# HKU-BAL/MegaPath-Nano

Measured on AMD Instinct MI355X. Metric: Gbp/min ONT reads aligned+species-assigned vs RefSeq, 1/2/4/8 MI355X, higher is better.
Workload: dtype int32

## Files before the change

### megapath_nano_amd/csrc/align.hip

```cpp
#include "map_types.h"
#include "ext_kernels.h"
#include "fin_kernels.h"
#include "tag_kernels.h"
#include "stitch_kernels.h"
#include "plan_kernels.h"
#include "hit_kernels.h"
#include "mapper_internal.h"
#include "../../include/mpn_map.h"
#include "../../include/mpn_ssw.h"

#include <algorithm>
#include <condition_variable>
#include <deque>
#include <math.h>
#include <stdio.h>
#include <string.h>
#include <thread>
#include <pthread.h>
#include <time.h>
#include <atomic>
#include <functional>
#include <mutex>
#include <stdlib.h>
#include <string>
// ... 629 lines not shown
                snprintf(buf, sizeof(buf), ",%d,%d;", q.mapq, q.blen - q.mlen + q.n_ambi);
                out += buf;
            }
        }
        if (r.has_p && o->with_cigar) write_diff_tags(o, r, out);
        snprintf(buf, sizeof(buf), "\trl:i:%d\n", rep_len);
        out += buf;
    }
}

struct Slot {
    hipEvent_t ev_b = nullptr, ev_c = nullptr;
    Arena arena;
    PoolBuf pool_jobs, pool_P, pool_P2, pool_OFF, pool_order, pool_state, pool_CIG, pool_res, pool_redo, pool_compact, pool_used;
    PoolBuf pool_redo_ids, pool_sregs, pool_souts, pool_fin_jobs, pool_fin_out, pool_fin_cig;
    PoolBuf pool_probes, pool_sizes, pool_buckets, pool_pregs, pool_psum, pool_job_anchor, pool_splits, pool_tags;
    PoolBuf pin_segs{nullptr, 0, true}, pin_pregs{nullptr, 0, true}, pin_hits{nullptr, 0, true};
    PoolBuf pin_order{nullptr, 0, true}, pin_res{nullptr, 0, true};
    PoolBuf pin_chain_u{nullptr, 0, true}, pin_chain_b{nullptr, 0, true};
    PoolBuf pin_fin_cig{nullptr, 0, true}, pin_fin_out{nullptr, 0, true}, pin_tags{nullptr, 0, true}, pin_tag_bytes{nullptr, 0, true};
    std::vector<std::vector<SqueezeSeg>> seg_stage;
    size_t device_bytes() const {
        size_t h = 0;
        for (const PoolBuf *pb : {&pool_jobs, &pool_P, &pool_P2, &pool_OFF, &pool_order, &pool_state, &pool_CIG, &pool_res, &pool_redo, &pool_compact, &pool_used,
                                  &pool_redo_ids, &pool_sregs, &pool_souts, &pool_fin_jobs, &pool_fin_out, &pool_fin_cig, &pool_probes, &pool_sizes, &pool_buckets,
                                  &pool_pregs, &pool_psum, &pool_job_anchor, &pool_splits, &pool_tags})
            h += pb->cap;
        for (const auto &c : arena.chunks) h += c.cap;
        return h;
    }
    void release_device() {
        arena.release_all();
        for (PoolBuf *pb : {&pool_jobs, &pool_P, &pool_P2, &pool_OFF, &pool_order, &pool_state, &pool_CIG, &pool_res, &pool_redo, &pool_compact, &pool_used,
                            &pool_redo_ids, &pool_sregs, &pool_souts, &pool_fin_jobs, &pool_fin_out, &pool_fin_cig, &pool_probes, &pool_sizes, &pool_buckets,
                            &pool_pregs, &pool_psum, &pool_job_anchor, &pool_splits, &pool_tags})
            pb->release();
    }
};
static Slot g_slots[16];
static thread_local Slot *tl_slot = &g_slots[0];

static int g_force_kernel = 0;

static void parallel_chunks(int64_t n, int n_threads, const std::function<void(int64_t, int64_t, int)> &fn, int tag = 0) {
    if (n_threads <= 1 || n < 8192) { fn(0, n, 0); return; }
    g_pool.parallel_for(n_threads, n_threads, [&](int t, int) { fn(n * t / n_threads, n * (t + 1) / n_threads, t); }, tag, 1);
}

__global__ void ext_redo_patch_kernel(ExtJob *jobs, const int32_t *ids, const int32_t *layout, const int32_t *qstride,
                                      const int64_t *p_off, const int32_t *inv, int zdrop_inv, int n) {
    const int k = blockIdx.x * blockDim.x + threadIdx.x;
    if (k >= n) return;
    ExtJob &jb = jobs[ids[k]];
    jb.flag &= ~EZ_APPROX_MAX;
    if (inv[k]) { jb.flag |= EZ_INV; jb.zdrop = zdrop_inv; }
    jb.layout = layout[k];
    jb.qstride = qstride[k];
    jb.p_off = p_off[k];
}

__global__ void ref_codes_kernel(RefView rv, const int64_t *g0, const int64_t *off, int n_iv, int8_t *out) {
    for (int k = blockIdx.y; k < n_iv; k += gridDim.y) {
        const int64_t n = off[k + 1] - off[k];
        for (int64_t i = (int64_t)blockIdx.x * blockDim.x + threadIdx.x; i < n; i += (int64_t)gridDim.x * blockDim.x)
            out[off[k] + i] = (int8_t)ref_code(rv, g0[k] + i);
    }
}
struct RefIv { int64_t seq_off; int start, n; };
static int fetch_ref_codes(const RefView &rv, const std::vector<RefIv> &iv, std::vector<std::vector<int8_t>> &out, StreamLease &st) {
    const int n_iv = (int)iv.size();
    out.resize((size_t)n_iv);
    if (n_iv == 0) return 0;
    std::vector<int64_t> tab((size_t)2 * n_iv + 1);
    int64_t *g0 = tab.data(), *off = g0 + n_iv;
    int max_n = 0;
    off[0] = 0;
    for (int k = 0; k < n_iv; ++k) {
        const int n = std::max(0, iv[(size_t)k].n);
        g0[k] = iv[(size_t)k].seq_off + iv[(size_t)k].start;
        off[k + 1] = off[k] + n;
        max_n = std::max(max_n, n);
    }
    const int64_t tot = off[n_iv];
    std::vector<int8_t> codes((size_t)tot);
    if (tot > 0) {
        DevBuf<int64_t> d_tab;
        DevBuf<int8_t> d;
        if (d_tab.alloc(tab.size()) || d.alloc((size_t)tot)) return -1;
        MPN_HIP_CHECK(hipMemcpyAsync(d_tab.p, tab.data(), tab.size() * 8, hipMemcpyHostToDevice, st));
        hipLaunchKernelGGL(ref_codes_kernel, dim3((unsigned)std::min(64, (max_n + 255) / 256), (unsigned)std::min(n_iv, 65535)), dim3(256), 0, st,
                           rv, (const int64_t *)d_tab.p, (const int64_t *)d_tab.p + n_iv, n_iv, d.p);
        MPN_HIP_CHECK(hipGetLastError());
        MPN_HIP_CHECK(hipMemcpyAsync(codes.data(), d.p, (size_t)tot, hipMemcpyDeviceToHost, st));
        MPN_HIP_CHECK(stream_sync(st));
    }
    for (int k = 0; k < n_iv; ++k) out[(size_t)k].assign(codes.begin() + off[k], codes.begin() + off[k + 1]);
    return 0;
}
static inline int8_t host_code(char c) { c |= 0x20; return c == 'a' ? 0 : c == 'c' ? 1 : c == 'g' ? 2 : (c == 't' || c == 'u') ? 3 : 4; }
static inline int8_t host_qbase(const char *seq, int rlen, int rev, int x) {
    if (!rev) return host_code(seq[x]);
    const int8_t c = host_code(seq[rlen - 1 - x]);
    return c < 4 ? (int8_t)(3 - c) : (int8_t)4;
}
struct LocalHit { int score, qe, te; };
static int local_scores(const mpn_map_opt *opt, const std::vector<std::vector<int8_t>> &qs, const std::vector<std::vector<int8_t>> &ts, std::vector<LocalHit> &out) {
    const int n = (int)qs.size();
    out.assign((size_t)n, LocalHit{0, -1, -1});
    if (n == 0) return 0;
    std::vector<int8_t> qb, tb;
    std::vector<int64_t> qo(n), to(n), coff(n);
    std::vector<int32_t> ql(n), tl(n), mask(n, 15), rb(n), re(n), qb1(n), qe1(n), re2(n), clen(n), status(n);
    std::vector<uint16_t> s1(n), s2(n);
    for (int i = 0; i < n; ++i) {
        qo[i] = (int64_t)qb.size(); ql[i] = (int32_t)qs[i].size(); qb.insert(qb.end(), qs[i].begin(), qs[i].end());
        to[i] = (int64_t)tb.size(); tl[i] = (int32_t)ts[i].size(); tb.insert(tb.end(), ts[i].begin(), ts[i].end());
    }
    int8_t mat[25];
    for (int i = 0; i < 4; ++i) { for (int j = 0; j < 4; ++j) mat[i * 5 + j] = (int8_t)(i == j ? opt->a : -opt->b); mat[i * 5 + 4] = (int8_t)-opt->sc_ambi; }
    for (int i = 0; i < 5; ++i) mat[20 + i] = (int8_t)-opt->sc_ambi;
    uint32_t dummy_cig[4];
    const int rc = mpn_ssw_align_batch(n, qb.data(), qo.data(), ql.data(), tb.data(), to.data(), tl.data(), mat, 5, 2, (uint8_t)(opt->q + opt->e), (uint8_t)opt->e,
                                       0, 0, 0, mask.data(), s1.data(), s2.data(), rb.data(), re.data(), qb1.data(), qe1.data(), re2.data(), dummy_cig, 4,
                                       coff.data(), clen.data(), status.data());
    if (rc) return -1;
    for (int i = 0; i < n; ++i) if (status[i] == 0) out[(size_t)i] = LocalHit{(int)s1[i], qe1[i], re[i]};
    return 0;
}

struct DevRound {
    ExtJob *jobs = nullptr;
    ExtRes *res = nullptr;
    uint32_t *compact = nullptr;
    unsigned long long *used = nullptr;
    int64_t cig_cap = 0;
    int n_jobs = 0;
};

struct HostSeqs { const char *seqs; const int64_t *seq_off; const int32_t *seq_len; const int64_t *tseq_off; };

static int run_job_group(const RefView &rv, const mpn_map_opt *opt, int nj_cap, const unsigned long long *d_nj, DevRound &dv, const uint8_t *d_reads,
                         const int64_t *d_read_off, const int32_t *d_read_len, int64_t budget, const HostSeqs *hs, StreamLease &st) {
    if (nj_cap == 0) return 0;
    int nj = nj_cap;
    WallTimer wt;
    Slot &SL = *tl_slot;
    const int strip_scores = ext_strip_scores_ok(opt->a, -opt->b, -opt->sc_ambi, opt->q + opt->e, opt->q2 + opt->e2) ? 1 : 0;
    ExtParams prm;
    prm.sc_mch = (int8_t)opt->a; prm.sc_mis = (int8_t)-opt->b; prm.sc_n = (int8_t)-opt->sc_ambi;
    prm.q = (int8_t)opt->q; prm.e = (int8_t)opt->e; prm.q2 = (int8_t)opt->q2; prm.e2 = (int8_t)opt->e2; prm.zdrop_thres = opt->zdrop;
    prm.zdrop_inv = opt->zdrop_inv; prm.max_gap = opt->max_gap;
    const size_t order_cap = (size_t)nj + (size_t)N_STRIP * 8 + 16;
    if (SL.pool_sizes.ensure((size_t)nj * sizeof(JobSizes) + 16) || SL.pool_buckets.ensure((size_t)2 * N_BUCKETS * 4 + sizeof(LayoutTotals) + 16) ||
        SL.pool_order.ensure(order_cap * 4) || SL.pin_res.ensure(sizeof(LayoutTotals) + 96) ||
        SL.pool_redo_ids.ensure((size_t)nj * 4 + 16) || SL.pool_probes.ensure((size_t)nj * sizeof(InvProbe) + 16))
        return -1;
    struct { ExtJob *p; } d_jobs{dv.jobs};
    JobSizes *d_sizes = SL.pool_sizes.as<JobSizes>();
    int32_t *d_bcnt = SL.pool_buckets.as<int32_t>(), *d_bcur = d_bcnt + N_BUCKETS;
    LayoutTotals *d_tot = reinterpret_cast<LayoutTotals *>(d_bcnt + 2 * N_BUCKETS);
    struct { int32_t *p; } d_order{SL.pool_order.as<int32_t>()};
    {
        ZeroList z{};
        zero_list_push(z, d_bcnt, (size_t)2 * N_BUCKETS * 4 + sizeof(LayoutTotals));
        zero_list_push(z, dv.used + 1, 8);
        zero_list_push(z, dv.used + 5, 8);
        zero_list_push(z, dv.used + 8, 16);
        zero_list_push(z, dv.used + 7, 8);
        MPN_HIP_CHECK(zero_regions(z, st));
    }
    const int lay_grid = std::max(1, std::min((nj + 255) / 256, 256));
    EvTimer evl(st);
    static const bool tiled_on = []() { const char *e = getenv("MPN_TILED"); return !e || atoi(e) != 0; }();
    static const int tile_pick = []() { const char *e = getenv("MPN_TILE_CLASS"); return e ? std::min(std::max(atoi(e), 0), N_TILE_CLASS - 1) : -1; }();
    hipLaunchKernelGGL(job_classify_kernel, dim3(lay_grid), dim3(256), 0, st, d_jobs.p, d_nj, strip_scores, prm, g_force_kernel ? g_force_kernel : (tiled_on ? 0 : 7),
                       tile_pick, d_sizes, d_bcnt, d_tot);
    hipLaunchKernelGGL(job_scan_kernel, dim3(1), dim3(1024), 0, st, d_sizes, d_nj, (const int32_t *)d_bcnt, d_bcur, d_tot, d_order.p);
    hipLaunchKernelGGL(job_layout_kernel, dim3(lay_grid), dim3(256), 0, st, d_jobs.p, d_nj, (const JobSizes *)d_sizes, d_bcur, d_order.p);
    MPN_HIP_CHECK(hipGetLastError());
    LayoutTotals *h_tot = SL.pin_res.as<LayoutTotals>();
    evl.mark(56);
    MPN_HIP_CHECK(hipMemcpyAsync(h_tot, d_tot, sizeof(LayoutTotals), hipMemcpyDeviceToHost, st));
    MPN_HIP_CHECK(stream_sync(st));
    evl.resolve();
    const LayoutTotals T = *h_tot;
    nj = T.n_jobs;
    dv.n_jobs = nj;
    if (nj == 0) return 0;
    if (T.too_large) { set_error("DP window too large for LDS staging (%d x %d)", T.tl_q, T.tl_t); return -4; }
    if (!dv.compact) {
        if (SL.pool_compact.ensure((size_t)T.cig_tot * 4 * 2 + 16)) return -1;
        dv.compact = SL.pool_compact.as<uint32_t>();
        dv.cig_cap = T.cig_tot;
    }
    if (budget > 0 && T.p_tot > budget && nj > 1) return 1;
    const int *cnt = T.cnt, *base = T.base;
    g_stats[4] += nj; g_stats[5] += T.cells; g_stats[31] += T.strip_cells[0] + T.strip_cells[1] + T.strip_cells[2];
    for (int c = 0; c < 3; ++c) g_stats[41 + c] += T.strip_cells[c];
    g_stats[58] += T.xstrip_cells;
    for (int c = 0; c < N_TILE_CLASS; ++c) {
        g_stats[64] += cnt[L_TILE + c];
        g_stats[STAT_TILE_CLASS + c] += cnt[L_TILE + c];
    }
    if (getenv("MPN_DEBUG_JOBS")) {
        static const char *const fam[] = {"wg64", "wg", "strip", "band", "tile"};
        for (int l = 0; l < N_LISTS; ++l)
            if (cnt[l]) fprintf(stderr, "[jobs] %s list %-2d n=%d\n", fam[l < L_WG ? 0 : l < L_STRIP ? 1 : l < L_BAND ? 2 : l < L_TILE ? 3 : 4], l, cnt[l]);
    }
    if (const char *dump = getenv("MPN_DUMP_STRIPS")) {
        const int n_ord = base[L_BAND] - base[L_STRIP];
        std::vector<int32_t> ord(n_ord);
        std::vector<ExtJob> hj(nj);
        MPN_HIP_CHECK(hipMemcpy(ord.data(), d_order.p + base[L_STRIP], (size_t)n_ord * 4, hipMemcpyDeviceToHost));
        MPN_HIP_CHECK(hipMemcpy(hj.data(), d_jobs.p, (size_t)nj * sizeof(ExtJob), hipMemcpyDeviceToHost));
        static std::mutex mu;
        std::lock_guard<std::mutex> lk(mu);
        if (const char *all = getenv("MPN_DUMP_JOBS"))
            if (FILE *f = fopen(all, "ab")) {
                for (int j = 0; j < nj; ++j) {
                    const int32_t rec[6] = {hj[j].cls, hj[j].qlen, hj[j].tlen, hj[j].w, hj[j].flag, hj[j].n_col};
                    fwrite(rec, 4, 6, f);
                }
                fclose(f);
            }
        if (FILE *f = fopen(dump, "ab")) {
            for (int l = L_STRIP; l < L_BAND; ++l)
                for (int k = base[l]; k < base[l + 1]; ++k) {
                    const int jid = ord[k - base[L_STRIP]];
                    const int32_t rec[4] = {strip_glc_of_list(l), jid >= 0 ? hj[jid].qlen : 0, jid >= 0 ? hj[jid].tlen : 0, jid >= 0 ? hj[jid].strip_s : 0};
                    fwrite(rec, 4, 4, f);
                }
            fclose(f);
        }
    }
    if (SL.pool_P.ensure((size_t)T.p_tot + 16) || SL.pool_OFF.ensure((size_t)T.row_tot * 2 * 4 + 16) ||
        SL.pool_state.ensure((size_t)T.state_tot + 16) || SL.pool_CIG.ensure((size_t)T.cig_tot * 4 + 16))
        return -1;
    wt.stop_into(g_stats[27]);
    struct { uint8_t *p; } P{SL.pool_P.as<uint8_t>()};
    struct { int32_t *p; } OFF{SL.pool_OFF.as<int32_t>()};
    struct { int8_t *p; } gstate{SL.pool_state.as<int8_t>()};
    struct { uint32_t *p; } CIG{SL.pool_CIG.as<uint32_t>()};
    struct { ExtRes *p; } d_res{dv.res};
    uint32_t *d_compact = dv.compact;
    unsigned long long *d_used = dv.used;
    int32_t *d_redo_ids = SL.pool_redo_ids.as<int32_t>();
    InvProbe *d_probes = SL.pool_probes.as<InvProbe>();
    auto launch_list = [&](int l, const int32_t *ord, int n, hipStream_t s) -> int {
        if (n == 0) return 0;
        if (l < L_STRIP) {
            const int ntc = (l - L_LDS) / 5;
            const size_t lds = std::max<size_t>((size_t)T.lds_need[(l - L_LDS) % 5], 64);
#define MPN_WG_LAUNCH(NT)                                                                                                             \
            do {                                                                                                                      \
                if (lds > 64 * 1024) MPN_HIP_CHECK(hipFuncSetAttribute((const void *)ext_dp_wg_kernel<NT>, hipFuncAttributeMaxDynamicSharedMemorySize, (int)lds)); \
                hipLaunchKernelGGL(ext_dp_wg_kernel<NT>, dim3(n), dim3(NT), lds, s, d_jobs.p, ord, n, prm, d_reads, d_read_off, d_read_len, \
                                   rv, P.p, OFF.p, gstate.p, d_res.p);                                                                \
            } while (0)
            if (ntc == 0) MPN_WG_LAUNCH(64); else if (ntc == 1) MPN_WG_LAUNCH(256); else if (ntc == 2) MPN_WG_LAUNCH(512); else MPN_WG_LAUNCH(1024);
#undef MPN_WG_LAUNCH
        } else if (l < L_BAND) {
            const int fam = (l - L_STRIP) / 48;
            StripSegs segs;
            segs.n = 0;
            int blocks = 0;
            size_t lds = 0;
            const int c_lo = fam == 0 ? 0 : 3, c_hi = fam == 0 ? 3 : N_STRIP_CLASS;
            for (int glc = 2; glc >= 0; --glc)
                for (int sclass = c_lo + glc; sclass < c_hi; sclass += 3) {
                    const int l0 = L_STRIP + 16 * sclass, nl = base[l0 + 16] - base[l0], per = strip_windows_per_wave(l0);
                    if (nl == 0) continue;
                    const int stride = (std::max(T.strip_lds[sclass], 16) + 3) & ~3;
                    const int nr_stride = fam ? T.strip_nr[sclass] + 16 : 0;
                    lds = std::max(lds, (size_t)stride * per + STRIP_TAB_BYTES + (size_t)per * 8 * nr_stride);
                    segs.s[segs.n++] = StripSeg{blocks, nl, base[l0], stride, nr_stride, glc, sclass >= 6 ? 1 : 0};
                    blocks += nl / per;
                }
            if (blocks == 0) return 0;
#define MPN_STRIP_LAUNCH(EX)                                                                                                          \
            do {                                                                                                                      \
                if (lds > 64 * 1024) MPN_HIP_CHECK(hipFuncSetAttribute((const void *)ext_dp_strip_kernel<EX>, hipFuncAttributeMaxDynamicSharedMemorySize, (int)lds)); \
                hipLaunchKernelGGL(ext_dp_strip_kernel<EX>, dim3(blocks), dim3(64), lds, s, d_jobs.p, (const int32_t *)d_order.p, segs, prm, d_reads, \
                                   d_read_off, d_read_len, rv, P.p, d_res.p);                                                         \
            } while (0)
            if (fam == 0) MPN_STRIP_LAUNCH(false); else MPN_STRIP_LAUNCH(true);
#undef MPN_STRIP_LAUNCH
        } else if (l >= L_TILE) {
            const int c = l - L_TILE;
            const size_t lds = (size_t)std::max(T.tile_lds[c], 64);
#define MPN_TILE_LAUNCH(S, NW)                                                                                                        \
            do {                                                                                                                      \
                if (lds > 64 * 1024) MPN_HIP_CHECK(hipFuncSetAttribute((const void *)ext_dp_tile_kernel<S, NW>, hipFuncAttributeMaxDynamicSharedMemorySize, (int)lds)); \
                hipLaunchKernelGGL((ext_dp_tile_kernel<S, NW>), dim3(n), dim3(64 * NW), lds, s, d_jobs.p, ord, n, prm, d_reads, d_read_off, \
                                   d_read_len, rv, P.p, gstate.p, d_res.p, d_used + 7);                                              \
            } while (0)
            static_assert(N_TILE_CLASS == 4, "tile classes");
            if (c == 0) MPN_TILE_LAUNCH(16, 1); else if (c == 1) MPN_TILE_LAUNCH(4, 8); else if (c == 2) MPN_TILE_LAUNCH(8, 4); else MPN_TILE_LAUNCH(4, 16);
#undef MPN_TILE_LAUNCH
        } else {
            const int bvar = (l - L_BAND) / 4;
            const size_t lds = std::max<size_t>((size_t)T.band_lds[(l - L_BAND) % 4], 64);
#define MPN_BAND_LAUNCH(NW, TT)                                                                                                       \
            do {                                                                                                                      \
                if (lds > 64 * 1024) MPN_HIP_CHECK(hipFuncSetAttribute((const void *)ext_dp_band_kernel<NW, TT>, hipFuncAttributeMaxDynamicSharedMemorySize, (int)lds)); \
                hipLaunchKernelGGL((ext_dp_band_kernel<NW, TT>), dim3(n), dim3(NW * 64), lds, s, d_jobs.p, ord, n, prm, d_reads, d_read_off, \
                                   d_read_len, rv, P.p, d_res.p);                                                                    \
            } while (0)
            if (bvar == 0) MPN_BAND_LAUNCH(1, 2); else if (bvar == 1) MPN_BAND_LAUNCH(2, 2); else if (bvar == 2) MPN_BAND_LAUNCH(4, 2); else MPN_BAND_LAUNCH(8, 2);
#undef MPN_BAND_LAUNCH
        }
        MPN_HIP_CHECK(hipGetLastError());
        return 0;
    };
    EvTimer ev(st);
    if (!SL.ev_b) {
        MPN_HIP_CHECK(hipEventCreateWithFlags(&SL.ev_b, hipEventDisableTiming));
        MPN_HIP_CHECK(hipEventCreateWithFlags(&SL.ev_c, hipEventDisableTiming));
    }
    auto on_side = [](int l) { return (l >= L_WG && l < L_STRIP) || l >= L_BAND + 8; };
    bool have_tiles = false;
    for (int l = L_TILE; l < N_LISTS; ++l) have_tiles = have_tiles || cnt[l] > 0;
    bool have_side = false;
    for (int l = 0; l < L_TILE; ++l) have_side = have_side || (on_side(l) && cnt[l] > 0);
    hipStream_t extra[2] = {nullptr, nullptr};
    const int n_extra = st.try_extra((int)have_side + (int)have_tiles, extra);
    if (have_side || have_tiles) ++g_stats[n_extra ? STAT_SIDE_LEASED : STAT_SIDE_OWN];
    const hipStream_t main_st = st;
    const hipStream_t side_st = have_side && n_extra > 0 ? extra[0] : main_st;
    const hipStream_t tile_st = have_tiles && n_extra > (int)have_side ? extra[(int)have_side] : main_st;
    for (int l = L_TILE; l < N_LISTS && have_tiles; ++l)
        if (launch_list(l, d_order.p + base[l], cnt[l], tile_st)) return -1;
    for (int l = L_TILE - 1; l >= 0; --l)
        if (on_side(l) && launch_list(l, d_order.p + base[l], cnt[l], side_st)) return -1;
    const int side_lo[2] = {base[L_WG], base[L_BAND + 8]}, side_hi[2] = {base[L_STRIP], base[L_TILE]};
    const int tile_lo[2] = {base[L_TILE], 0}, tile_hi[2] = {base[N_LISTS], 0};
    const int main_lo[2] = {0, base[L_STRIP]}, main_hi[2] = {base[L_WG], base[L_BAND + 8]};
    static const int walk_mode = []() {
        const char *e = getenv("MPN_EXT_WALK");
        return !e || !strcmp(e, "auto") ? 0 : !strcmp(e, "lane") ? 1 : !strcmp(e, "wave") ? 2 : 0;
    }();
    auto launch_bt = [&](const int32_t *ord, int n, hipStream_t s, bool wave) {
        if (n <= 0) return;
        if (wave) hipLaunchKernelGGL(ext_bt_wave_kernel, dim3(n), dim3(64), 0, s, d_jobs.p, ord, n, P.p, OFF.p, CIG.p, d_compact, d_used, d_res.p, d_used + 8);
        else hipLaunchKernelGGL(ext_bt_kernel, dim3((n + 63) / 64), dim3(64), 0, s, d_jobs.p, ord, n, P.p, OFF.p, CIG.p, d_compact, d_used, d_res.p);
    };
    auto bt_ztest = [&](const int *lo, const int *hi, hipStream_t s, bool timed, bool wave) -> int {
        for (int k = 0; k < 2; ++k) launch_bt(d_order.p + lo[k], hi[k] - lo[k], s, wave);
        MPN_HIP_CHECK(hipGetLastError());
        if (timed) ev.mark(25);
        for (int k = 0; k < 2; ++k) {
            const int n = hi[k] - lo[k];
            if (n <= 0) continue;
            if (wave) hipLaunchKernelGGL(ext_ztest_wave_kernel, dim3(n), dim3(64), 0, s, d_jobs.p, d_order.p + lo[k], n, prm, d_reads, d_read_off, d_read_len, rv, CIG.p, d_res.p,
                                         d_redo_ids, d_used + 1, d_probes, d_used + 5, d_used + 9);
            else hipLaunchKernelGGL(ext_ztest_kernel, dim3((n + 63) / 64), dim3(64), 0, s, d_jobs.p, d_order.p + lo[k], n, prm, d_reads, d_read_off, d_read_len, rv, CIG.p, d_res.p,
                                    d_redo_ids, d_used + 1, d_probes, d_used + 5);
        }
        MPN_HIP_CHECK(hipGetLastError());
        if (timed) ev.mark(26);
        return 0;
    };
    if (have_side || have_tiles) ev.mark(15);
    if (have_tiles) {
        if (bt_ztest(tile_lo, tile_hi, tile_st, false, walk_mode != 1)) return -1;
        if (tile_st != main_st) MPN_HIP_CHECK(hipEventRecord(SL.ev_c, tile_st));
    }
    if (bt_ztest(side_lo, side_hi, side_st, false, walk_mode != 1)) return -1;
    if (side_st != main_st) MPN_HIP_CHECK(hipEventRecord(SL.ev_b, side_st));
    if (have_side || have_tiles) ev.mark(STAT_EV_WALK_LONG);
    for (int l = N_LISTS - 1; l >= 0; --l) {
        if (on_side(l)) continue;
        if (l == L_BAND - 1) ev.mark(15);
        if (l >= L_STRIP && l < L_BAND) {
            if (l == L_STRIP + 48) { if (launch_list(l, nullptr, 1, main_st)) return -1; ev.mark(57); }
            else if (l == L_STRIP) { if (launch_list(l, nullptr, 1, main_st)) return -1; ev.mark(9, 38); }
        } else if (launch_list(l, d_order.p + base[l], cnt[l], main_st)) return -1;
    }
    ev.mark(15);
    if (bt_ztest(main_lo, main_hi, main_st, true, walk_mode == 2)) return -1;
    if (side_st != main_st) MPN_HIP_CHECK(hipStreamWaitEvent(main_st, SL.ev_b, 0));
    if (tile_st != main_st) MPN_HIP_CHECK(hipStreamWaitEvent(main_st, SL.ev_c, 0));
    unsigned long long *h_used = reinterpret_cast<unsigned long long *>(reinterpret_cast<char *>(SL.pin_res.p) + ((sizeof(LayoutTotals) + 15) & ~(size_t)15));
    MPN_HIP_CHECK(hipMemcpyAsync(h_used, d_used, 80, hipMemcpyDeviceToHost, st));
    wt.stop_into(g_stats[28]);
    MPN_HIP_CHECK(stream_sync(st));
    wt.stop_into(g_stats[29]);
    g_stats[STAT_WALK_WAVE] += (int64_t)h_used[8];
    g_stats[STAT_WALK_WAVE_FAILED] += (int64_t)h_used[9];
    if (h_used[7]) {
        g_stats[STAT_TILE_GIVEUPS] += (int64_t)h_used[7];
        set_error("%llu tiled DP windows gave up waiting for their hand-off", (unsigned long long)h_used[7]);
        return -1;
    }
    std::vector<int32_t> redo((size_t)h_used[1]);
    const int n_probe = (int)h_used[5];
    if (!redo.empty() || n_probe) {
        std::vector<ExtJob> jobs((size_t)nj);
        std::vector<InvProbe> probes((size_t)n_probe);
        if (SL.pin_order.ensure(redo.size() * 4 + 16)) return -1;
        if (!redo.empty()) MPN_HIP_CHECK(hipMemcpyAsync(SL.pin_order.p, d_redo_ids, redo.size() * 4, hipMemcpyDeviceToHost, st));
        MPN_HIP_CHECK(hipMemcpyAsync(jobs.data(), d_jobs.p, (size_t)nj * sizeof(ExtJob), hipMemcpyDeviceToHost, st));
        if (n_probe) MPN_HIP_CHECK(hipMemcpyAsync(probes.data(), d_probes, (size_t)n_probe * sizeof(InvProbe), hipMemcpyDeviceToHost, st));
        MPN_HIP_CHECK(stream_sync(st));
        if (!redo.empty()) memcpy(redo.data(), SL.pin_order.p, redo.size() * 4);
        std::vector<uint8_t> is_inv((size_t)nj, 0);
        if (n_probe) {
            std::sort(probes.begin(), probes.end(), [](const InvProbe &x, const InvProbe &y) { return x.jid < y.jid; });
            std::vector<LocalHit> hits((size_t)n_probe, LocalHit{0, -1, -1});
            if (hs) {
                std::vector<std::vector<int8_t>> qv((size_t)n_probe), tv;
                std::vector<RefIv> iv((size_t)n_probe);
                for (int k = 0; k < n_probe; ++k) {
                    const InvProbe &pb = probes[(size_t)k];
                    const ExtJob &jb = jobs[(size_t)pb.jid];
                    const int q_len = pb.q1 - pb.q0, t_len = pb.t1 - pb.t0, rlen = hs->seq_len[jb.read];
                    const char *rd = hs->seqs + hs->seq_off[jb.read];
                    qv[(size_t)k].resize((size_t)q_len);
                    for (int x = 0; x < q_len; ++x) { const int8_t c = host_qbase(rd, rlen, jb.rev, jb.qs + pb.q1 - x - 1); qv[(size_t)k][(size_t)x] = c >= 4 ? (int8_t)4 : (int8_t)(3 - c); }
                    iv[(size_t)k] = RefIv{hs->tseq_off[jb.rid], jb.ts + pb.t0, t_len};
                }
                if (fetch_ref_codes(rv, iv, tv, st)) return -1;
                if (local_scores(opt, qv, tv, hits)) return -1;
            }
            for (int k = 0; k < n_probe; ++k) {
                const InvProbe &pb = probes[(size_t)k];
                const bool inv = hits[(size_t)k].score >= opt->min_chain_score * opt->a && hits[(size_t)k].score >= opt->min_dp_max;
                if (inv) is_inv[(size_t)pb.jid] = 1;
                if (inv || pb.over) redo.push_back(pb.jid);
            }
        }
        g_stats[8] += (int64_t)redo.size();
        const int nr = (int)redo.size();
        auto list_of = [&](int j) { return jobs[(size_t)j].cls & 0xff; };
        auto redo_list_of = [&](int j) { return jobs[(size_t)j].cls >> 8 & 0xff; };
        auto band_of = [&](int j) { return (jobs[(size_t)j].cls >> 16 & 0xff) - 1; };
        std::sort(redo.begin(), redo.end(), [&](int x, int y) { return redo_list_of(x) != redo_list_of(y) ? redo_list_of(x) < redo_list_of(y) : x < y; });
        std::vector<int32_t> pack((size_t)nr * 6 + 2);
        const size_t off_p = ((size_t)nr * 4 + 1) & ~(size_t)1;
        int64_t *pack_off = reinterpret_cast<int64_t *>(pack.data() + off_p);
        int64_t p2_tot = 0;
        for (int k = 0; k < nr; ++k) {
            const int j = redo[k];
            const ExtJob &jb = jobs[(size_t)j];
            const int bv = band_of(j);
            pack[k] = j; pack[nr + k] = bv >= 0 ? 2 : 0; pack[2 * nr + k] = 128 << std::max(bv, 0); pack[3 * nr + k] = is_inv[(size_t)j];
            if ((list_of(j) >= L_STRIP && list_of(j) < L_BAND) || list_of(j) >= L_TILE) {
                const int64_t n_r = (int64_t)jb.qlen + jb.tlen - 1;
                pack_off[k] = -1 - p2_tot;
                p2_tot += ((bv >= 0 ? n_r * (128 << bv) : n_r * jb.n_col) + 15) & ~(int64_t)15;
            } else pack_off[k] = jb.p_off;
        }
        if (nr > 0) {
            if (SL.pool_P2.ensure((size_t)p2_tot + 16)) return -1;
            const int64_t p2_base = (int64_t)(SL.pool_P2.as<uint8_t>() - P.p);
            for (int k = 0; k < nr; ++k) if (pack_off[k] < 0) pack_off[k] = p2_base + (-1 - pack_off[k]);
            if (SL.pool_redo.ensure(pack.size() * 4)) return -1;
            struct { int32_t *p; } d_redo{SL.pool_redo.as<int32_t>()};
            MPN_HIP_CHECK(hipMemcpyAsync(d_redo.p, pack.data(), pack.size() * 4, hipMemcpyHostToDevice, st));
            hipLaunchKernelGGL(ext_redo_patch_kernel, dim3((nr + 255) / 256), dim3(256), 0, st, d_jobs.p, d_redo.p, d_redo.p + nr, d_redo.p + 2 * nr,
                               reinterpret_cast<const int64_t *>(d_redo.p + off_p), d_redo.p + 3 * nr, opt->zdrop_inv, nr);
            MPN_HIP_CHECK(hipGetLastError());
            ev.skip();
            for (int lo = 0; lo < nr;) {
                int hi = lo;
                while (hi < nr && redo_list_of(redo[hi]) == redo_list_of(redo[lo])) ++hi;
                if (launch_list(redo_list_of(redo[lo]), d_redo.p + lo, hi - lo, st)) return -1;
                lo = hi;
            }
            ev.mark(15);
            launch_bt(d_redo.p, nr, st, walk_mode == 2);
            if (walk_mode == 2) g_stats[STAT_WALK_WAVE] += nr;
            MPN_HIP_CHECK(hipGetLastError());
            ev.mark(25);
            MPN_HIP_CHECK(stream_sync(st));
        }
    }
    ev.resolve();
    wt.stop_into(g_stats[30]);
    return 0;
}

static int run_jobs(const RefView &rv, const mpn_map_opt *opt, int nj_cap, const uint8_t *d_reads, const int64_t *d_read_off,
                    const int32_t *d_read_len, DevRound &out, const HostSeqs *hs, StreamLease &st, bool block_zeroed = false) {
    static const int64_t budget = []() { const char *e = getenv("MPN_DP_BUDGET"); return e ? std::max<int64_t>(1 << 20, atoll(e)) : (int64_t)40 << 30; }();
    Slot &SL = *tl_slot;
    if (SL.pool_res.ensure((size_t)nj_cap * sizeof(ExtRes) + 16) || SL.pool_used.ensure(128)) return -1;
    out.jobs = SL.pool_jobs.as<ExtJob>(); out.res = SL.pool_res.as<ExtRes>(); out.compact = nullptr;
    out.used = SL.pool_used.as<unsigned long long>();
    if (!block_zeroed) {
        MPN_HIP_CHECK(hipMemsetAsync(out.used, 0, 24, st));
        MPN_HIP_CHECK(hipMemsetAsync(out.used + 5, 0, 24, st));
    }
    const int rc = run_job_group(rv, opt, nj_cap, out.used + 3, out, d_reads, d_read_off, d_read_len, budget, hs, st);
    if (rc != 1) return rc;
    const int nj = out.n_jobs;
    std::vector<JobSizes> sz((size_t)nj);
    MPN_HIP_CHECK(hipMemcpyAsync(sz.data(), SL.pool_sizes.p, (size_t)nj * sizeof(JobSizes), hipMemcpyDeviceToHost, st));
    MPN_HIP_CHECK(stream_sync(st));
    std::vector<int> cuts{0};
    for (int j = 1; j < nj; ++j) if (sz[(size_t)j].p - sz[(size_t)cuts.back()].p > budget) cuts.push_back(j);
    cuts.push_back(nj);
    for (size_t g = 0; g + 1 < cuts.size(); ++g) {
        DevRound dv = out;
        dv.jobs += cuts[g]; dv.res += cuts[g];
        const unsigned long long cnt = (unsigned long long)(cuts[g + 1] - cuts[g]);
        MPN_HIP_CHECK(hipMemcpyAsync(out.used + 4, &cnt, 8, hipMemcpyHostToDevice, st));
        const int r2 = run_job_group(rv, opt, (int)cnt, out.used + 4, dv, d_reads, d_read_off, d_read_len, 0, hs, st);
        if (r2) return r2 < 0 ? r2 : -1;
    }
    out.n_jobs = nj;
    return 0;
}

}

using namespace mpn;

static int plan_enqueue(const mpn_map_opt *opt, int32_t k, const PlanReg *d_pr, int n_sr, u128 *d_a, const int32_t *d_tlens,
                        unsigned long long *d_used, ExtJob *d_jobs, int32_t *d_janchor, StitchReg *d_sr, PlanSum *d_ps, int grid_cap,
                        hipStream_t st) {
    PlanOpt po;
    po.bw = opt->bw; po.bw15 = (int)(opt->bw * 1.5 + 1.); po.min_chain_score = opt->min_chain_score; po.max_gap = opt->max_gap;
    po.min_cnt = opt->min_cnt; po.a = opt->a; po.q = opt->q; po.e = opt->e; po.zdrop = opt->zdrop; po.zdrop_inv = opt->zdrop_inv;
    po.end_bonus = opt->end_bonus; po.min_ksw_len = opt->min_ksw_len; po.k = k; po.pad = 0; po.max_sw_mat = opt->max_sw_mat;
    MPN_HIP_CHECK(hipMemsetAsync(d_used, 0, 64, st));
    int grid = std::min(n_sr, 256 * 4);
    if (grid_cap > 0) grid = std::min(grid, grid_cap);
    hipLaunchKernelGGL(plan_kernel, dim3((unsigned)grid), dim3(64), 0, st, po, d_pr, n_sr, d_a, d_tlens, d_used + 3, d_jobs, d_janchor, d_sr, d_ps);
    MPN_HIP_CHECK(hipGetLastError());
    return 0;
}

static bool g_need_cigar = true;

struct RoundDev {
    const StitchReg *sregs; const PlanReg *pregs; const PlanSum *psum; const int32_t *job_anchor; const u128 *anchors;
};

static int stitch_enqueue(const RoundDev &rd, int n_sr, const ExtJob *d_jobs, const ExtRes *d_res, const uint32_t *d_compact, uint32_t *d_cig,
                          unsigned long long *d_out_used, StitchOut *d_so, FinJob *d_fj, int min_cnt, SplitRec *d_splits,
                          unsigned long long *d_n_splits, int grid_cap, hipStream_t st) {
// ... 1840 lines not shown
```

### megapath_nano_amd/csrc/ext_kernels.h

```cpp
#pragma once
#include "mpn_common.h"
#include "map_types.h"

namespace mpn {

enum { EZ_APPROX_MAX = 0x02, EZ_RIGHT = 0x08, EZ_EXTZ_ONLY = 0x40, EZ_REV_CIGAR = 0x80 };

struct ExtJob {
    int32_t read;
    int32_t rid;
    int32_t rev;
    int32_t qs, qlen;
    int32_t ts, tlen;
    int32_t reversed;
    int32_t w, zdrop, end_bonus, flag;
    int64_t p_off;
    int64_t row_off;
    int64_t cig_off;
    int32_t n_col;
    int32_t state_mode;
    int64_t state_off;
    int32_t layout;
    int32_t qstride;
    int32_t strip_s;
// ... 752 lines not shown
        uint32_t Vp = ((uint32_t)v_s & nh) | (((uint32_t)bj * both + CV) & ~nh), X1 = (uint32_t)x1_s & nh, X2 = (uint32_t)x2_s & nh;
        if (j >= 0 && j < qmax && gl < nlmax) {
            uint32_t dwa[(S + 3) / 4], dwb[(S + 3) / 4], ecell[4] = {0, 0, 0, 0};
            uint32_t nv0 = 0;
#pragma unroll
            for (int k = 0; k < S; ++k) {
                const uint32_t sc = __builtin_amdgcn_perm(qta, KONST, T1[k]) | __builtin_amdgcn_perm(qtb, KONST, T2[k]);
                const uint32_t Up = U[k];
                const uint32_t A1 = X1 + Vp, A2 = X2 + Vp, B1 = Y1[k] + Up, B2 = Y2[k] + Up;
                const uint32_t M1 = __builtin_bit_cast(uint32_t, __builtin_elementwise_max(__builtin_bit_cast(s16x2, A1), __builtin_bit_cast(s16x2, B1)));
                const uint32_t M2 = __builtin_bit_cast(uint32_t, __builtin_elementwise_max(__builtin_bit_cast(s16x2, A2), __builtin_bit_cast(s16x2, B2))) - DD;
                const uint32_t M = __builtin_bit_cast(uint32_t, __builtin_elementwise_max(__builtin_bit_cast(s16x2, M1), __builtin_bit_cast(s16x2, M2)));
                const uint32_t z = __builtin_bit_cast(uint32_t, __builtin_elementwise_max(__builtin_bit_cast(s16x2, M), __builtin_bit_cast(s16x2, sc)));
                const uint32_t zc = __builtin_bit_cast(uint32_t, __builtin_elementwise_min(__builtin_bit_cast(s16x2, z), __builtin_bit_cast(s16x2, MCH7)));
                const uint32_t Zc = zc & RANK_CLR;
                const uint32_t ZZ = Zc + KZZ;
                uint32_t nu = Up, nv;
                asm("v_sub_u32 %1, %2, %0\n\tv_sub_u32 %0, %2, %3" : "+v"(nu), "=&v"(nv) : "v"(ZZ), "v"(Vp));
                const u16x2 An1 = __builtin_elementwise_sub_sat(__builtin_bit_cast(u16x2, A1), __builtin_bit_cast(u16x2, Zc + KEA1));
                const u16x2 An2 = __builtin_elementwise_sub_sat(__builtin_bit_cast(u16x2, A2), __builtin_bit_cast(u16x2, Zc + KEA2));
                const u16x2 Bn1 = __builtin_elementwise_sub_sat(__builtin_bit_cast(u16x2, B1), __builtin_bit_cast(u16x2, Zc + KEB1));
                const u16x2 Bn2 = __builtin_elementwise_sub_sat(__builtin_bit_cast(u16x2, B2), __builtin_bit_cast(u16x2, Zc + KEB2));
                uint32_t HA1, HB1, HA2, HB2, F;
                asm("v_pk_min_u16 %0, %1, %2" : "=v"(HA1) : "v"(__builtin_bit_cast(uint32_t, An1)), "v"(EIGHT));
                asm("v_pk_min_u16 %0, %1, %2" : "=v"(HB1) : "v"(__builtin_bit_cast(uint32_t, Bn1)), "v"(EIGHT));
                asm("v_pk_min_u16 %0, %1, %2" : "=v"(HA2) : "v"(__builtin_bit_cast(uint32_t, An2)), "v"(EIGHT));
                asm("v_pk_min_u16 %0, %1, %2" : "=v"(HB2) : "v"(__builtin_bit_cast(uint32_t, Bn2)), "v"(EIGHT));
                asm("v_lshl_or_b32 %0, %1, 1, %2" : "=v"(F) : "v"(HB1), "v"(HA1));
                asm("v_lshl_or_b32 %0, %1, 2, %2" : "=v"(F) : "v"(HA2), "v"(F));
                asm("v_lshl_or_b32 %0, %1, 3, %2" : "=v"(F) : "v"(HB2), "v"(F));
                asm("v_and_or_b32 %0, %1, %2, %3" : "=v"(ecell[k & 3]) : "v"(z), "v"(SEVEN), "v"(F));
                U[k] = nu; Y1[k] = __builtin_bit_cast(uint32_t, Bn1); Y2[k] = __builtin_bit_cast(uint32_t, Bn2);
                Vp = nv; X1 = __builtin_bit_cast(uint32_t, An1); X2 = __builtin_bit_cast(uint32_t, An2);
                if ((k & 3) == 3 || k == S - 1) {
                    const uint32_t p01 = (k & 3) >= 1 ? __builtin_amdgcn_perm(ecell[1], ecell[0], 0x06020400u) : __builtin_amdgcn_perm(0u, ecell[0], 0x0c020c00u);
                    const uint32_t p23 = (k & 3) == 3 ? __builtin_amdgcn_perm(ecell[3], ecell[2], 0x06020400u)
                                       : (k & 3) == 2 ? __builtin_amdgcn_perm(0u, ecell[2], 0x0c020c00u) : 0u;
                    dwa[k >> 2] = __builtin_amdgcn_perm(p23, p01, 0x05040100u);
                    dwb[k >> 2] = __builtin_amdgcn_perm(p23, p01, 0x07060302u);
                }
                if (k == 0) nv0 = nv;
            }
            out_v = (int)Vp; out_x1 = (int)X1; out_x2 = (int)X2;
            if (j <= qa1) row0a += (int)(nv0 & 0xffffu) - cv1;
            if (j <= qb1) row0b += (int)(nv0 >> 16) - cv1;
            auto packed_sum = [&]() -> uint32_t {
                u16x2 acc = __builtin_bit_cast(u16x2, U[0]);
#pragma unroll
                for (int k = 1; k < S; ++k) acc += __builtin_bit_cast(u16x2, U[k]);
                return __builtin_bit_cast(uint32_t, acc);
            };
            if (j == qa1) {
                if (!head && t0 + S <= tlen[0]) tota += (int)(short)(uint16_t)((packed_sum() & 0xffffu) - (uint32_t)(S * cu1));
                else {
#pragma unroll
                    for (int k = 0; k < S; ++k) tota += (t0 + k > 0 && t0 + k < tlen[0]) ? (int)(U[k] & 0xffffu) - cu1 : 0;
                }
            }
            if (j == qb1) {
                if (!head && t0 + S <= tlen[1]) totb += (int)(short)(uint16_t)((packed_sum() >> 16) - (uint32_t)(S * cu1));
                else {
#pragma unroll
                    for (int k = 0; k < S; ++k) totb += (t0 + k > 0 && t0 + k < tlen[1]) ? (int)(U[k] >> 16) - cu1 : 0;
                }
            }
            auto store = [&](uint8_t *dst, const uint32_t *dw) {
                if constexpr (S == 4) *reinterpret_cast<uint32_t *>(dst) = dw[0];
                else if constexpr (S == 8) *reinterpret_cast<uint2 *>(dst) = make_uint2(dw[0], dw[1]);
                else if constexpr (S == 16) *reinterpret_cast<uint4 *>(dst) = make_uint4(dw[0], dw[1], dw[2], dw[3]);
                else {
#pragma unroll
                    for (int c = 0; c < S / 4; ++c) __builtin_memcpy(dst + 4 * c, &dw[c], 4);
                    if constexpr ((S & 2) != 0) { const uint16_t h = (uint16_t)dw[S / 4]; __builtin_memcpy(dst + (S & ~3), &h, 2); }
                    if constexpr ((S & 1) != 0) dst[S - 1] = (uint8_t)(dw[S / 4] >> ((S & 2) ? 16 : 0));
                }
            };
            if (j <= qa1 && gl < nl0) store(prow0 + (int64_t)step * W[0], dwa);
            if (j <= qb1 && gl < nl1) store(prow1 + (int64_t)step * W[1], dwb);
        }
    }
#undef MPN_BND
    int32_t ta = tota + (head ? row0a - 8 * qe : 0), tb = totb + (head ? row0b - 8 * qe : 0);
#pragma unroll
    for (int dlt = GL / 2; dlt; dlt >>= 1) { ta += __shfl_xor(ta, dlt); tb += __shfl_xor(tb, dlt); }
    ta >>= 3; tb >>= 3;
    if (head) {
#pragma unroll
        for (int w = 0; w < 2; ++w) {
            if (jid[w] < 0) continue;
            ExtRes out;
            out.max = 0; out.zdropped = 0; out.max_q = out.max_t = out.mqe_t = -1; out.mqe = NEG_INF; out.score = ok[w] ? (w ? tb : ta) : NEG_INF;
            out.reach_end = 0; out.n_cigar = 0; out.r_done = ok[w] ? qlen[w] + tlen[w] - 2 : -1; out.zcode = 0; out.cig_pos = 0;
            out.do_bt = ok[w] ? 1 : 0; out.bt_i = ok[w] ? tlen[w] - 1 : -1; out.bt_j = ok[w] ? qlen[w] - 1 : -1;
            res[jid[w]] = out;
        }
    }
}

template <int GL, bool RIGHT>
__device__ __forceinline__ void ext_strip_exact_dispatch(const ExtJob *__restrict__ jobs, const int32_t *__restrict__ order, const int first,
                                                         const int n_list, const ExtParams &prm, const uint8_t *__restrict__ reads,
                                                         const int64_t *__restrict__ read_off, const int32_t *__restrict__ read_len,
                                                         const RefView &rv, uint8_t *__restrict__ P, ExtRes *__restrict__ res, uint8_t *smem,
                                                         const int lds_stride, const int nr_stride) {
    const int j0 = first < n_list ? order[first] : -1;
    if (j0 < 0) return;
    const int S = jobs[j0].strip_s;
#define MPN_CASE(SS) case SS: ext_strip_exact<SS, GL, RIGHT>(jobs, order, first, n_list, prm, reads, read_off, read_len, rv, P, res, smem, lds_stride, nr_stride); break
    switch (S) {
        MPN_CASE(1); MPN_CASE(2); MPN_CASE(3); MPN_CASE(4); MPN_CASE(5); MPN_CASE(6); MPN_CASE(7); MPN_CASE(8);
        MPN_CASE(9); MPN_CASE(10); MPN_CASE(11); MPN_CASE(12); MPN_CASE(13); MPN_CASE(14); MPN_CASE(15);
        default: ext_strip_exact<16, GL, RIGHT>(jobs, order, first, n_list, prm, reads, read_off, read_len, rv, P, res, smem, lds_stride, nr_stride); break;
    }
#undef MPN_CASE
}

struct StripSeg { int32_t first_block, n_list, ord_off, lds_stride, nr_stride, glc, right; };
struct StripSegs { StripSeg s[6]; int32_t n; };

template <bool EXACT>
__global__ __launch_bounds__(64) __attribute__((amdgpu_waves_per_eu(3, 3))) void ext_dp_strip_kernel(const ExtJob *__restrict__ jobs, const int32_t *__restrict__ order, StripSegs segs,
                                                          ExtParams prm, const uint8_t *__restrict__ reads,
                                                          const int64_t *__restrict__ read_off, const int32_t *__restrict__ read_len,
                                                          RefView rv, uint8_t *__restrict__ P, ExtRes *__restrict__ res) {
    extern __shared__ __attribute__((aligned(16))) uint8_t smem[];
    int k = 0;
    while (k + 1 < segs.n && (int)blockIdx.x >= segs.s[k + 1].first_block) ++k;
    const StripSeg sg = segs.s[k];
    const int32_t *ord = order + sg.ord_off;
    if constexpr (!EXACT) {
        {
            const int first2 = ((int)blockIdx.x - sg.first_block) * (8 >> sg.glc);
            int S = 16;
            for (int k = 0; k < (8 >> sg.glc); ++k) { const int slot = first2 + k; if (slot < sg.n_list && ord[slot] >= 0) { S = jobs[ord[slot]].strip_s; break; } }
#define MPN_PAIR(SS, GLN) ext_strip_pair<SS, GLN>(jobs, ord, first2, sg.n_list, prm, reads, read_off, read_len, rv, P, res, smem, sg.lds_stride)
#define MPN_PAIR_S(GLN) switch (S) { case 1: MPN_PAIR(1, GLN); break; case 2: MPN_PAIR(2, GLN); break; case 3: MPN_PAIR(3, GLN); break; case 4: MPN_PAIR(4, GLN); break; \
            case 5: MPN_PAIR(5, GLN); break; case 6: MPN_PAIR(6, GLN); break; case 7: MPN_PAIR(7, GLN); break; case 8: MPN_PAIR(8, GLN); break; \
            case 9: MPN_PAIR(9, GLN); break; case 10: MPN_PAIR(10, GLN); break; case 11: MPN_PAIR(11, GLN); break; case 12: MPN_PAIR(12, GLN); break; \
            case 13: MPN_PAIR(13, GLN); break; case 14: MPN_PAIR(14, GLN); break; case 15: MPN_PAIR(15, GLN); break; default: MPN_PAIR(16, GLN); break; }
            if (sg.glc == 0) MPN_PAIR_S(16) else if (sg.glc == 1) MPN_PAIR_S(32) else MPN_PAIR_S(64)
#undef MPN_PAIR_S
#undef MPN_PAIR
        }
    } else {
        const int first = ((int)blockIdx.x - sg.first_block) * (4 >> sg.glc);
#define MPN_GL(GLN, RT) ext_strip_exact_dispatch<GLN, RT>(jobs, ord, first, sg.n_list, prm, reads, read_off, read_len, rv, P, res, smem, sg.lds_stride, sg.nr_stride)
        if (sg.right) { if (sg.glc == 0) MPN_GL(16, true); else if (sg.glc == 1) MPN_GL(32, true); else MPN_GL(64, true); }
        else { if (sg.glc == 0) MPN_GL(16, false); else if (sg.glc == 1) MPN_GL(32, false); else MPN_GL(64, false); }
#undef MPN_GL
    }
}

struct TileGeom { int T0, rows, n_lanes, W, jlo, jhi; int64_t base; };
__host__ __device__ inline TileGeom tile_geom(int tile, int qlen, int tlen, int w, int S) {
    const int R = 64 * S;
    TileGeom g{};
    g.T0 = tile * R;
    g.rows = tlen - g.T0 < R ? tlen - g.T0 : R;
    g.n_lanes = (g.rows + S - 1) / S;
    g.W = g.n_lanes * S;
    g.jlo = g.T0 - w > 0 ? g.T0 - w : 0;
    g.jhi = g.T0 + g.rows - 1 + w < qlen - 1 ? g.T0 + g.rows - 1 + w : qlen - 1;
    const int64_t m = tile;
    const int64_t k0 = (int64_t)w / R + 1;
    const int64_t n0 = m > k0 ? m - k0 : 0;
    const int64_t s_lo = (int64_t)R * (n0 * (k0 + m - 1) / 2) - n0 * (int64_t)w;
    const int64_t num = (int64_t)qlen - R - w;
    int64_t k1 = num <= 0 ? 0 : (num + R - 1) / R;
    if (k1 > m) k1 = m;
    const int64_t s_hi = (int64_t)R * (k1 * (k1 - 1) / 2) + k1 * (int64_t)(R - 1 + w) + (m - k1) * (int64_t)(qlen - 1);
    g.base = (s_hi - s_lo + 64 * m) * R;
    return g;
}
__host__ __device__ inline int64_t tile_matrix_bytes(int qlen, int tlen, int w, int S) {
    const int R = 64 * S, nt_all = (tlen + R - 1) / R, nt_band = (int)(((int64_t)qlen - 1 + w) / R) + 1, nt = nt_all < nt_band ? nt_all : nt_band;
    const TileGeom g = tile_geom(nt - 1, qlen, tlen, w, S);
    return g.base + (int64_t)((g.jhi >= g.jlo ? g.jhi - g.jlo + 1 : 0) + g.n_lanes - 1) * g.W;
}
__host__ __device__ inline bool ext_tile_ok(int qlen, int tlen, int w) {
    const int d = qlen > tlen ? qlen - tlen : tlen - qlen;
    return qlen > 0 && tlen > 0 && w >= 1 && d <= w && tlen <= 32768 && qlen <= 60000;
}

__host__ __device__ inline bool ext_tile_exact_ok(int mch, int mis, int amb, int q, int e, int q2, int e2, int qlen, int tlen, int w) {
    if (!(qlen > 0 && tlen > 0 && w >= 1 && tlen <= 8191 && qlen <= 16384 && qlen + tlen - 1 <= 14000)) return false;
    const int mn = qlen < tlen ? qlen : tlen, mx = qlen > tlen ? qlen : tlen;
    int worst = mis < amb ? -mis : -amb;
    if (worst < 0) worst = 0;
    const int g1 = worst * mn + q + e * (mx - mn + 1), g1b = q + e * (mx + 1), g2 = worst * mn + q2 + e2 * (mx - mn + 1), g2b = q2 + e2 * (mx + 1);
    const int lo1 = g1 > g1b ? g1 : g1b, lo2 = g2 > g2b ? g2 : g2b;
    return mch * mn < 32000 && (lo1 < lo2 ? lo1 : lo2) < 32000;
}
constexpr int TILE_RING_COLS = 2048, TILE_CTRL_BYTES = 4 * (2 * 16 + 4);
__host__ __device__ inline int ext_tile_ring_off(int qlen) { return ((qlen + 3) & ~3) + 64 + TILE_CTRL_BYTES; }
__host__ __device__ inline int ext_tile_lds_bytes(int qlen, int tlen, bool exact, int NW) {
    return ext_tile_ring_off(qlen) + (NW > 1 ? 12 * TILE_RING_COLS : 0) + (exact ? 8 * ((qlen + tlen + 2) & ~3) : 0);
}
__host__ __device__ inline bool ext_tile_pipe_ok(int w, int S, int NW) {
    return 2 * w + 128 < NW * (TILE_RING_COLS / NW + 64 * S);
}
constexpr int TILE_SPIN_MAX = 1 << 21;

template <int S, int NW, bool EXACT, bool RIGHT>
__device__ __forceinline__ void ext_tile_body(const ExtJob &jb, const int jid, const ExtParams &prm, const uint8_t *__restrict__ reads,
                                              const int64_t *__restrict__ read_off, const int32_t *__restrict__ read_len, const RefView &rv,
                                              uint8_t *__restrict__ P, int8_t *__restrict__ gstate, ExtRes *__restrict__ res, uint8_t *smem,
                                              unsigned long long *__restrict__ n_failed) {
    static_assert(S % 4 == 0 && S <= 16 && NW >= 1 && NW <= 16, "rows per lane: 4, 8, 12 or 16");
    constexpr int R = 64 * S, NT = 64 * NW;
    const int tid = threadIdx.x, lane = tid & 63, wave = tid >> 6;
    const int qlen = jb.qlen, tlen = jb.tlen;
    int q = prm.q, e = prm.e, q2 = prm.q2, e2 = prm.e2;
    if (q2 + e2 < q + e) { int t_ = q; q = q2; q2 = t_; t_ = e; e = e2; e2 = t_; }
    const int qe = q + e, qe2 = q2 + e2;
    int w = jb.w;
    if (w < 0) w = tlen > qlen ? tlen : qlen;
    ExtRes out;
    out.max = 0; out.zdropped = 0; out.max_q = out.max_t = out.mqe_t = -1; out.mqe = NEG_INF; out.score = NEG_INF;
    out.reach_end = 0; out.n_cigar = 0; out.r_done = -1; out.bt_i = out.bt_j = -1; out.do_bt = 0; out.zcode = 0; out.cig_pos = 0;
    if (!(EXACT ? ext_tile_exact_ok(prm.sc_mch, prm.sc_mis, prm.sc_n, prm.q, prm.e, prm.q2, prm.e2, qlen, tlen, w) : ext_tile_ok(qlen, tlen, w)) || -prm.sc_mis > 2 * (q + e) ||
        (NW > 1 && !ext_tile_pipe_ok(w, S, NW))) { if (tid == 0) res[jid] = out; return; }
    constexpr int RS = RIGHT ? 0 : 4, RA = RIGHT ? 1 : 3, RB = 2, RA2 = RIGHT ? 3 : 1, RB2 = RIGHT ? 4 : 0;
    const uint32_t sb_mch = (uint32_t)(8 * prm.sc_mch + RS + 128) & 0xff, sb_mis = (uint32_t)(8 * prm.sc_mis + RS + 128) & 0xff,
                   sb_n = (uint32_t)(8 * prm.sc_n + RS + 128) & 0xff;
    const int q_pad = (qlen + 3) & ~3;
    uint32_t *tab = reinterpret_cast<uint32_t *>(smem + q_pad);
    if (tid < 5) tab[tid] = lane == 4 ? sb_n * 0x01010101u : (sb_mis * 0x01010101u) ^ ((sb_mch ^ sb_mis) << (8 * lane));
    {
        const int64_t roff = read_off[jb.read];
        const int32_t rlen = read_len[jb.read];
        for (int i = tid; i < qlen; i += NT) smem[i] = (uint8_t)(4 * ext_qbase(reads, roff, rlen, jb.rev, jb.qs + (jb.reversed ? qlen - 1 - i : i)));
    }
    int long_thres = e != e2 ? (q2 - q) / (e - e2) - 1 : 0;
    if (q2 + e2 + long_thres * e2 > q + e + long_thres * e) ++long_thres;
    const int long_diff = long_thres * (e - e2) - (q2 - q) - e2;
#define MPN_BND(R) (8 * ((R) == 0 ? -qe : (R) < long_thres ? -e : (R) == long_thres ? long_diff : -e2))
    typedef short s16x2 __attribute__((ext_vector_type(2)));
    typedef unsigned short u16x2 __attribute__((ext_vector_type(2)));
    auto pk = [](int lo, int hi) { return (uint32_t)(hi * 65536 + lo); };
    constexpr int BETA = 0x2000 + 128;
    const int cv_lo = -8 * qe + RA + BETA, cv_hi = -8 * qe2 + RA2 + BETA, cu_lo = -8 * qe + RB + BETA, cu_hi = -8 * qe2 + RB2 + BETA;
    const uint32_t CV = pk(cv_lo, cv_hi), CU = pk(cu_lo, cu_hi);
    const uint32_t FRESH_U = pk(-8 * qe, -8 * qe) + CU, EDGE_V = pk(-8 * qe, -8 * qe) + CV;
    const uint32_t KONST = sb_n | 0x2000u;
    const uint32_t KZZ = pk(-16 * qe + RA + RB + BETA, -16 * qe2 + RA2 + RB2 + BETA);
    constexpr int RU = RIGHT ? 8 : 0;
    const uint32_t KEA = pk(8 * e - 8 * qe + RA - RU, 8 * e2 - 8 * qe2 + RA2 - RU), KEB = pk(8 * e - 8 * qe + RB - RU, 8 * e2 - 8 * qe2 + RB2 - RU);
    const uint32_t EIGHT = 0x00080008u, RANK_CLR = 0xfff8fff8u;
    const uint32_t MCH7 = (uint32_t)(8 * prm.sc_mch + 7 + BETA) * 0x00010001u;
    const int64_t g0 = rv.seq_off[jb.rid] + jb.ts;
    uint32_t *bnd_base = reinterpret_cast<uint32_t *>(gstate + jb.state_off);
    const int n_tiles = (tlen + R - 1) / R;
    uint32_t *ctrl = reinterpret_cast<uint32_t *>(smem + ext_tile_ring_off(qlen) - TILE_CTRL_BYTES);
    uint32_t *ring = ctrl + TILE_CTRL_BYTES / 4;
    constexpr int C = TILE_RING_COLS / NW;
    const int n_r = qlen + tlen - 1;
    uint32_t *BEST = reinterpret_cast<uint32_t *>(smem + ext_tile_ring_off(qlen) + (NW > 1 ? 12 * TILE_RING_COLS : 0)), *SE = BEST + ((n_r + 3) & ~3);
    int32_t *HL = reinterpret_cast<int32_t *>(NW > 1 ? bnd_base : bnd_base + 6 * (size_t)qlen);
    if (tid < 2 * NW + 1) ctrl[tid] = 0;
    if constexpr (EXACT) {
        for (int r = tid; r < n_r; r += NT) {
            int st = 0, en = tlen - 1;
            if (st < r - qlen + 1) st = r - qlen + 1;
            if (en > r) en = r;
            if (st < (r - w + 1) >> 1) st = (r - w + 1) >> 1;
            if (en > (r + w) >> 1) en = (r + w) >> 1;
            if (st > en) { st = 1; en = 0; }
            BEST[r] = 0;
            SE[r] = (uint32_t)st | (uint32_t)en << 16;
        }
        for (int t = tid; t < tlen; t += NT) HL[t] = NEG_INF;
        __builtin_amdgcn_fence(__ATOMIC_RELEASE, "agent");
    }
    __syncthreads();
    const bool head = lane == 0;
    int32_t score8 = 0;
    uint32_t *const prod_in = &ctrl[(wave + NW - 1) % NW], *const cons_in = &ctrl[NW + (wave + NW - 1) % NW];
    uint32_t *const prod_out = &ctrl[wave], *const cons_out = &ctrl[NW + wave];
    uint32_t *const ring_in = ring + 3 * C * ((wave + NW - 1) % NW), *const ring_out = ring + 3 * C * wave;
    uint32_t n_in = 0, n_out = 0, seen_prod = 0, seen_cons = 0;
    bool failed = false;
    auto wait_gt = [&](uint32_t *ctr, uint32_t lim, uint32_t &seen) -> bool {
        if ((int)(seen - lim) > 0) return true;
        for (int k = 0; k < TILE_SPIN_MAX; ++k) {
            seen = __hip_atomic_load(ctr, __ATOMIC_RELAXED, __HIP_MEMORY_SCOPE_WORKGROUP);
            if ((int)(seen - lim) > 0) return true;
            if (__hip_atomic_load(&ctrl[2 * NW], __ATOMIC_RELAXED, __HIP_MEMORY_SCOPE_WORKGROUP)) return false;
            __builtin_amdgcn_s_sleep(1);
        }
        __hip_atomic_store(&ctrl[2 * NW], 1u, __ATOMIC_RELAXED, __HIP_MEMORY_SCOPE_WORKGROUP);
        return false;
    };
    for (int tile = NW > 1 ? wave : 0; tile < n_tiles; tile += NW) {
        const TileGeom G = tile_geom(tile, qlen, tlen, w, S);
        const int T0 = G.T0, n_lanes = G.n_lanes, W = G.W, jlo = G.jlo, jhi = G.jhi;
        if (jhi < jlo) break;
        const int prev_jhi = tile > 0 ? min(qlen - 1, T0 - 1 + w) : -1;
        const int jlo_next = T0 + R - w > 0 ? T0 + R - w : 0;
        uint32_t *bnd_in = bnd_base + (size_t)(tile & 1) * 3 * (size_t)qlen, *bnd_out = bnd_base + (size_t)((tile + 1) & 1) * 3 * (size_t)qlen;
        const bool write_bnd = tile + 1 < n_tiles;
        const int t0 = T0 + lane * S;
        uint32_t UL[S], YL[S], TSEL[S];
        int32_t H8[S];
#pragma unroll
        for (int k = 0; k < S; ++k) {
            const int t = t0 + k;
            const int sq = t < tlen ? ref_code(rv, g0 + (jb.reversed ? tlen - 1 - t : t)) : 4;
            TSEL[k] = 0x0c0c0100u | (sq < 4 ? 4u + (uint32_t)sq : 0u);
            UL[k] = jlo == 0 ? pk(MPN_BND(t), MPN_BND(t)) + CU : FRESH_U;
            YL[k] = 0;
            H8[k] = 8 * (t < long_thres ? -(q + e * (t + 1)) : -(q2 + e2 * (t + 1)));
        }
        uint8_t *prow = P + jb.p_off + G.base + (int64_t)lane * S;
        const int n_steps = (jhi - jlo + 1) + n_lanes - 1;
        int out_v = 0, out_x = 0, out_h = 0;
        uint32_t qt = 0;
        auto qcode = [&](int col) -> uint32_t { return col < qlen ? (uint32_t)smem[col] : 16u; };
        uint32_t qt_next = *reinterpret_cast<const uint32_t *>(reinterpret_cast<const uint8_t *>(tab) + qcode(jlo));
        uint32_t qc_next = qcode(jlo + 1);
        uint32_t bv_n = 0, bx_n = 0, bh_n = 0, bv_n2 = 0, bx_n2 = 0, bh_n2 = 0;
        auto load_bnd = [&](int col, uint32_t &a, uint32_t &b, uint32_t &c) {
            if (tile > 0 && head && col <= prev_jhi && col < qlen) {
                if constexpr (NW == 1) { a = bnd_in[3 * (size_t)col]; b = bnd_in[3 * (size_t)col + 1]; c = bnd_in[3 * (size_t)col + 2]; }
                else {
                    const uint32_t n = n_in + (uint32_t)(col - jlo), slot = n % C;
                    if (!failed && !wait_gt(prod_in, n, seen_prod)) failed = true;
                    __atomic_signal_fence(__ATOMIC_SEQ_CST);
                    a = ring_in[slot]; b = ring_in[C + slot]; c = ring_in[2 * C + slot];
                    __atomic_signal_fence(__ATOMIC_SEQ_CST);
                    __hip_atomic_store(cons_in, n + 1, __ATOMIC_RELAXED, __HIP_MEMORY_SCOPE_WORKGROUP);
                }
            }
        };
        load_bnd(jlo, bv_n, bx_n, bh_n);
        load_bnd(jlo + 1, bv_n2, bx_n2, bh_n2);
        for (int step = 0; step < n_steps; ++step) {
            const uint32_t q_in = qt_next;
            qt_next = *reinterpret_cast<const uint32_t *>(reinterpret_cast<const uint8_t *>(tab) + qc_next);
            qc_next = qcode(jlo + step + 2);
            const uint32_t bv = bv_n, bx = bx_n, bh = bh_n;
            bv_n = bv_n2; bx_n = bx_n2; bh_n = bh_n2;
            load_bnd(jlo + step + 2, bv_n2, bx_n2, bh_n2);
            const uint32_t qt_s = (uint32_t)wave_shr1_zero((int)qt);
            const int v_s = wave_shr1_zero(out_v), x_s = wave_shr1_zero(out_x), h_s = wave_shr1_zero(out_h);
            const int j = jlo + step - lane;
            qt = head ? q_in : qt_s;
            uint32_t Vp, Xp;
            int32_t Hup;
            if (head) {
                if (tile == 0) { const int bj = MPN_BND(j); Vp = pk(bj, bj) + CV; Xp = 0; Hup = 0; }
                else { Vp = bv; Xp = bx; Hup = (int32_t)bh; }
            } else { Vp = (uint32_t)v_s; Xp = (uint32_t)x_s; Hup = h_s; }
            if (j >= jlo && j <= jhi && lane < n_lanes) {
                uint32_t dw[S / 4], ecell[4] = {0, 0, 0, 0};
                const int d_in = j - t0 + w;
                const int d_out = j - t0 - w;
#pragma unroll
                for (int k = 0; k < S; ++k) {
                    const bool enter = d_in == k, edge = d_out == k;
                    const uint32_t Up = enter ? FRESH_U : UL[k];
                    const uint32_t Yl = enter ? 0u : YL[k];
                    Vp = edge ? EDGE_V : Vp;
                    Xp = edge ? 0u : Xp;
                    const uint32_t sc16 = __builtin_amdgcn_perm(qt, KONST, TSEL[k]);
                    const uint32_t A = Xp + Vp, B = Yl + Up;
                    const uint32_t M = __builtin_bit_cast(uint32_t, __builtin_elementwise_max(__builtin_bit_cast(s16x2, A), __builtin_bit_cast(s16x2, B)));
                    uint32_t m2, z16;
                    asm("v_pk_max_i16 %0, %1, %1 op_sel:[0,1] op_sel_hi:[1,0]" : "=v"(m2) : "v"(M));
                    asm("v_max_i16 %0, %1, %2" : "=v"(z16) : "v"(m2), "v"(sc16));
                    uint32_t zc;
                    asm("v_pk_min_i16 %0, %1, %2 op_sel_hi:[0,1]" : "=v"(zc) : "v"(z16), "v"(MCH7));
                    const uint32_t Zc = zc & RANK_CLR;
                    const uint32_t ZZ = Zc + KZZ;
                    const uint32_t nu = ZZ - Vp, nv = ZZ - Up;
                    u16x2 An = __builtin_elementwise_sub_sat(__builtin_bit_cast(u16x2, A), __builtin_bit_cast(u16x2, Zc + KEA));
                    u16x2 Bn = __builtin_elementwise_sub_sat(__builtin_bit_cast(u16x2, B), __builtin_bit_cast(u16x2, Zc + KEB));
                    uint32_t HA, HB;
                    asm("v_pk_min_u16 %0, %1, %2" : "=v"(HA) : "v"(__builtin_bit_cast(uint32_t, An)), "v"(EIGHT));
                    asm("v_pk_min_u16 %0, %1, %2" : "=v"(HB) : "v"(__builtin_bit_cast(uint32_t, Bn)), "v"(EIGHT));
                    if constexpr (RIGHT) {
                        An = __builtin_elementwise_sub_sat(An, __builtin_bit_cast(u16x2, EIGHT));
                        Bn = __builtin_elementwise_sub_sat(Bn, __builtin_bit_cast(u16x2, EIGHT));
                    }
                    uint32_t Fw;
                    asm("v_lshl_or_b32 %0, %1, 1, %2" : "=v"(Fw) : "v"(HB), "v"(HA));
                    asm("v_and_or_b32 %0, %1, 7, %2" : "=v"(ecell[k & 3]) : "v"(z16), "v"(Fw));
                    const int32_t h_left = H8[k] + (int32_t)(nv & 0xffffu) - cv_lo, h_up = Hup + (int32_t)(nu & 0xffffu) - cu_lo;
                    const int32_t h = enter ? h_up : h_left;
                    H8[k] = h;
                    Hup = h;
                    if constexpr (EXACT) {
                        const int t = t0 + k, r = t + j;
                        const uint32_t se = SE[r < n_r ? r : n_r - 1];
                        const int st_ = (int)(se & 0xffffu), en_ = (int)(se >> 16);
                        const bool inb = t >= st_ && t <= en_;
                        const int en1 = st_ + ((en_ - st_) & ~3);
                        const int cls = t == en_ ? 0 : t < en1 ? 1 + ((t - st_) & 3) : 5;
                        const uint32_t word = (uint32_t)((h >> 3) + 32768) << 16 | (0xffffu - ((uint32_t)cls << 13 | (uint32_t)t));
                        atomicMax(&BEST[r < n_r ? r : n_r - 1], inb ? word : 0u);
                        if (inb && j == qlen - 1) HL[t] = h >> 3;
                    }
                    UL[k] = nu; YL[k] = __builtin_bit_cast(uint32_t, Bn);
                    Vp = nv; Xp = __builtin_bit_cast(uint32_t, An);
                    if ((k & 3) == 3) {
                        uint32_t e01, e23;
                        asm("v_lshl_or_b32 %0, %1, 8, %2" : "=v"(e01) : "v"(ecell[1]), "v"(ecell[0]));
                        asm("v_lshl_or_b32 %0, %1, 8, %2" : "=v"(e23) : "v"(ecell[3]), "v"(ecell[2]));
                        const uint32_t lo = __builtin_amdgcn_perm(e23, e01, 0x05040100u), hi = __builtin_amdgcn_perm(e23, e01, 0x07060302u);
                        asm("v_lshl_or_b32 %0, %1, 2, %2" : "=v"(dw[k >> 2]) : "v"(hi), "v"(lo));
                    }
                }
                out_v = (int)Vp; out_x = (int)Xp; out_h = Hup;
                if constexpr (S == 16) *reinterpret_cast<uint4 *>(prow + (int64_t)step * W) = make_uint4(dw[0], dw[1], dw[2], dw[3]);
                else if constexpr (S == 8) *reinterpret_cast<uint2 *>(prow + (int64_t)step * W) = make_uint2(dw[0], dw[1]);
                else if constexpr (S == 4) *reinterpret_cast<uint32_t *>(prow + (int64_t)step * W) = dw[0];
                if constexpr (NW == 1) {
                    if (write_bnd && lane == 63) { bnd_out[3 * (size_t)j] = (uint32_t)out_v; bnd_out[3 * (size_t)j + 1] = (uint32_t)out_x; bnd_out[3 * (size_t)j + 2] = (uint32_t)out_h; }
                } else if (write_bnd && lane == 63 && j >= jlo_next) {
                    const uint32_t n = n_out + (uint32_t)(j - jlo_next), slot = n % C;
                    if (!failed && !wait_gt(cons_out, n - C, seen_cons)) failed = true;
                    __atomic_signal_fence(__ATOMIC_SEQ_CST);
                    ring_out[slot] = (uint32_t)out_v; ring_out[C + slot] = (uint32_t)out_x; ring_out[2 * C + slot] = (uint32_t)out_h;
                    __atomic_signal_fence(__ATOMIC_SEQ_CST);
                    __hip_atomic_store(prod_out, n + 1, __ATOMIC_RELAXED, __HIP_MEMORY_SCOPE_WORKGROUP);
                }
            }
        }
        if (tile + 1 == n_tiles) {
            const int lt = tlen - 1 - T0, ll = lt / S, kk = lt % S;
            int32_t hv = 0;
#pragma unroll
            for (int k = 0; k < S; ++k) hv = k == kk ? H8[k] : hv;
            score8 = __shfl(hv, ll);
        }
        if constexpr (NW == 1) {
            __builtin_amdgcn_fence(__ATOMIC_RELEASE, "agent");
            __syncthreads();
            __builtin_amdgcn_fence(__ATOMIC_ACQUIRE, "agent");
        } else {
            if (tile > 0 && prev_jhi >= jlo) n_in += (uint32_t)(prev_jhi - jlo + 1);
            if (write_bnd && jhi >= jlo_next) n_out += (uint32_t)(jhi - jlo_next + 1);
        }
    }
#undef MPN_BND
    if constexpr (NW > 1) {
        __builtin_amdgcn_fence(__ATOMIC_RELEASE, "agent");
        __syncthreads();
        __builtin_amdgcn_fence(__ATOMIC_ACQUIRE, "agent");
        if (wave != (EXACT ? 0 : (n_tiles - 1) % NW)) return;
        if (__hip_atomic_load(&ctrl[2 * NW], __ATOMIC_RELAXED, __HIP_MEMORY_SCOPE_WORKGROUP)) {
            if (lane == 0) { res[jid] = out; atomicAdd(n_failed, 1ull); }
            return;
        }
    }
    if constexpr (!EXACT) {
        if (lane == 0) {
            out.score = score8 >> 3;
            out.r_done = qlen + tlen - 2;
            out.do_bt = 1; out.bt_i = tlen - 1; out.bt_j = qlen - 1;
            res[jid] = out;
        }
    } else {
        if constexpr (NW == 1) __syncthreads();
        const int tlm1 = tlen - 1;
        struct Best { int m, t, r; };
        auto scan_first_max = [&](Best x) {
#pragma unroll
            for (int d = 1; d < 64; d <<= 1) {
                const Best o{__shfl_up(x.m, d), __shfl_up(x.t, d), __shfl_up(x.r, d)};
                if (lane >= d && !(x.m > o.m)) x = o;
            }
            return x;
        };
        auto diag = [&](int r, int &H, int &mt) {
            const uint32_t pv = BEST[r];
            H = pv ? (int)(pv >> 16) - 32768 : NEG_INF;
            mt = (int)((0xffffu - (pv & 0xffffu)) & 8191u);
        };
        int r_lim = n_r;
        for (int r = lane; r < n_r; r += 64) { const uint32_t se = SE[r]; if ((int)(se & 0xffffu) > (int)(se >> 16)) { r_lim = r; break; } }
        r_lim = wave_reduce_min(r_lim);
        const int n_eff = r_lim < n_r ? r_lim : n_r;
        const int C = (n_eff + 63) / 64, rlo = min(n_eff, lane * C), rhi = min(n_eff, rlo + C);
        auto chunk_best = [&](int lim) {
            Best b{NEG_INF, -1, -1};
            for (int r = rlo; r < rhi && r <= lim; ++r) { int H, mt; diag(r, H, mt); if (H > b.m) b = Best{H, mt, r}; }
            return b;
        };
        Best incl = scan_first_max(chunk_best(n_eff));
        Best in{__shfl_up(incl.m, 1), __shfl_up(incl.t, 1), __shfl_up(incl.r, 1)};
        ExtApply ez; ez.max = 0; ez.max_t = ez.max_q = -1; ez.zdropped = 0;
        if (lane > 0 && in.m > 0) { ez.max = in.m; ez.max_t = in.t; ez.max_q = in.r - in.t; }
        int r_break = n_eff;
        for (int r = rlo; r < rhi; ++r) {
            int H, mt; diag(r, H, mt);
            if (ext_apply_zdrop(ez, H, r, mt, jb.zdrop, e2)) { r_break = r; break; }
        }
        r_break = wave_reduce_min(r_break);
        const bool zd = r_break < n_eff;
        const bool dropped = zd || n_eff < n_r;
        const int r_last = zd ? r_break : n_eff - 1;
        Best fin = scan_first_max(chunk_best(r_last));
        fin = Best{__shfl(fin.m, 63), __shfl(fin.t, 63), __shfl(fin.r, 63)};
        __builtin_amdgcn_fence(__ATOMIC_ACQUIRE, "agent");
        const int t_lim = min(tlm1, r_last - (qlen - 1));
        const int Ct = (tlen + 63) / 64, tlo = min(tlen, lane * Ct), thi = min(tlen, tlo + Ct);
        Best me{NEG_INF, -1, -1};
        for (int t = tlo; t < thi && t <= t_lim; ++t) { const int h = HL[t]; if (h > me.m) me = Best{h, t, t}; }
        me = scan_first_max(me);
        me = Best{__shfl(me.m, 63), __shfl(me.t, 63), 0};
        if (lane == 0) {
            if (fin.m > 0) { out.max = fin.m; out.max_t = fin.t; out.max_q = fin.r - fin.t; }
            out.zdropped = dropped ? 1 : 0;
            if (me.m > NEG_INF) { out.mqe = me.m; out.mqe_t = me.t; }
            if (!dropped) out.score = HL[tlm1];
            out.r_done = dropped ? (zd ? r_break : n_eff) : n_r - 1;
            if (!dropped && !(jb.flag & EZ_EXTZ_ONLY)) { out.do_bt = 1; out.bt_i = tlen - 1; out.bt_j = qlen - 1; }
            else if (!dropped && (jb.flag & EZ_EXTZ_ONLY) && out.mqe + jb.end_bonus > out.max) { out.reach_end = 1; out.do_bt = 1; out.bt_i = out.mqe_t; out.bt_j = qlen - 1; }
            else if (out.max_t >= 0 && out.max_q >= 0) { out.do_bt = 1; out.bt_i = out.max_t; out.bt_j = out.max_q; }
            res[jid] = out;
        }
    }
}

template <int S, int NW>
__global__ __launch_bounds__(64 * NW) void ext_dp_tile_kernel(const ExtJob *__restrict__ jobs, const int32_t *__restrict__ order, int n_jobs,
                                                              ExtParams prm, const uint8_t *__restrict__ reads,
                                                              const int64_t *__restrict__ read_off, const int32_t *__restrict__ read_len,
                                                              RefView rv, uint8_t *__restrict__ P, int8_t *__restrict__ gstate, ExtRes *__restrict__ res,
                                                              unsigned long long *__restrict__ n_failed) {
    extern __shared__ __attribute__((aligned(16))) uint8_t smem[];
    const int jid = order[blockIdx.x];
    const ExtJob jb = jobs[jid];
#define MPN_TB(EX, RT) ext_tile_body<S, NW, EX, RT>(jb, jid, prm, reads, read_off, read_len, rv, P, gstate, res, smem, n_failed)
    if (jb.flag & EZ_APPROX_MAX) MPN_TB(false, false);
    else if (jb.flag & EZ_RIGHT) MPN_TB(true, true);
    else MPN_TB(true, false);
#undef MPN_TB
}



__device__ __forceinline__ void ext_bt_band(int rr, int qlen, int tlen, int bw, int &st, int &en) {
    st = 0; en = tlen - 1;
    if (st < rr - qlen + 1) st = rr - qlen + 1;
    if (en > rr) en = rr;
    if (st < (rr - bw + 1) >> 1) st = (rr - bw + 1) >> 1;
    if (en > (rr + bw) >> 1) en = (rr + bw) >> 1;
}
__device__ __forceinline__ int ext_bt_force(int i, int st, int en) {
    int force_state = -1;
    if (i < st) force_state = 2;
    if (i > en) force_state = 1;
    return force_state;
}
__device__ __forceinline__ int ext_bt_decode(int b, bool rank_is_op) { return rank_is_op ? b : (b & ~7) | (4 - (b & 7)); }
__device__ __forceinline__ int ext_bt_next_state(int state, int tmp, int force_state) {
    if (state == 0) state = tmp & 7;
    else if (!(tmp >> (state + 2) & 1)) state = 0;
    if (state == 0) state = tmp & 7;
    if (force_state >= 0) state = force_state;
    return state;
}

__global__ __launch_bounds__(64) void ext_bt_kernel(const ExtJob *__restrict__ jobs, const int32_t *__restrict__ order, int n_jobs,
                                                    const uint8_t *__restrict__ P, const int32_t *__restrict__ OFF,
                                                    uint32_t *__restrict__ CIG, uint32_t *__restrict__ COMPACT,
                                                    unsigned long long *__restrict__ compact_used, ExtRes *__restrict__ res) {
    const int k = blockIdx.x * blockDim.x + threadIdx.x;
    const int jid = k < n_jobs ? order[k] : -1;
    const bool live = jid >= 0;
    ExtJob jb = jobs[live ? jid : 0];
    ExtRes r = res[live ? jid : 0];
    const bool walk = live && r.do_bt;
    if (live && !r.do_bt) res[jid].cig_pos = 0;
    if (!walk) { jb.qlen = jb.tlen = 1; r.bt_i = r.bt_j = -1; }
    const int n_col = jb.n_col, n_r = jb.qlen + jb.tlen - 1;
    const uint8_t *p = P + jb.p_off;
    const int32_t *off = OFF + 2 * jb.row_off, *off_end = off + n_r;
    const bool rowmajor = jb.layout == 1;
    const bool rank_is_op = (jb.flag & EZ_RIGHT) != 0;
    const bool byslot = jb.layout == 2;
    const bool tiled = jb.layout == 3;
    TileGeom tg{};
    int tg_tile = -1;
    const int bw = jb.w < 0 ? (jb.tlen > jb.qlen ? jb.tlen : jb.qlen) : jb.w;
    const bool rev_cigar = (jb.flag & EZ_REV_CIGAR) != 0;
    uint32_t *cend = CIG + jb.cig_off;
    const int cap = jb.qlen + jb.tlen + 2;
    uint32_t *cbeg = cend - cap;
    int n = 0, i = r.bt_i, j = r.bt_j, state = 0;
    uint32_t cur_op = 0xf, cur_len = 0;
#define MPN_FLUSH() do { if (cur_len) { if (rev_cigar) cbeg[n] = cur_len << 4 | cur_op; else cend[-1 - n] = cur_len << 4 | cur_op; ++n; } } while (0)
#define MPN_PUSHOP(OP, LEN) do { if ((uint32_t)(OP) == cur_op) cur_len += (LEN); else { MPN_FLUSH(); cur_op = (OP); cur_len = (LEN); } } while (0)
    constexpr int BT_AHEAD = 8;
    while (i >= 0 && j >= 0) {
        const int rr = i + j;
        int force_state = -1, tmp;
        if (rowmajor) {
            if (state == 0) {
                uint8_t ahead[BT_AHEAD];
#pragma unroll
                for (int k = 0; k < BT_AHEAD; ++k) {
                    const int ii = i - k, jj = j - k;
                    ahead[k] = (ii >= 0 && jj >= 0) ? p[(int64_t)(jj + ii / jb.strip_s) * jb.qstride + ii] : (uint8_t)0xff;
                }
                int k = 0;
                tmp = 0;
#pragma unroll
                for (int q = 0; q < BT_AHEAD; ++q) {
                    if (k != q) continue;
                    if (i - q < 0 || j - q < 0) continue;
                    const int b = ext_bt_decode(ahead[q], rank_is_op);
                    if ((b & 7) == 0) ++k; else tmp = b;
                }
                if (k > 0) { MPN_PUSHOP(0, (uint32_t)k); i -= k; j -= k; }
                if (k == BT_AHEAD || i < 0 || j < 0) continue;
            } else {
                tmp = ext_bt_decode(p[(int64_t)(j + i / jb.strip_s) * jb.qstride + i], rank_is_op);
            }
        }
        else if (tiled) {
            int st, en;
            ext_bt_band(rr, jb.qlen, jb.tlen, bw, st, en);
            force_state = ext_bt_force(i, st, en);
            tmp = 0;
            if (force_state < 0) {
                const int tile = i / (64 * jb.strip_s);
                if (tile != tg_tile) { tg = tile_geom(tile, jb.qlen, jb.tlen, bw, jb.strip_s); tg_tile = tile; }
                const int lt = i - tg.T0;
                tmp = ext_bt_decode(p[tg.base + (int64_t)((j - tg.jlo) + lt / jb.strip_s) * tg.W + lt], rank_is_op);
            }
        }
        else if (byslot) {
            int st, en;
            ext_bt_band(rr, jb.qlen, jb.tlen, bw, st, en);
            force_state = ext_bt_force(i, st, en);
            tmp = force_state < 0 ? p[(int64_t)rr * jb.qstride + (i & (jb.qstride - 1))] : 0;
        } else {
            force_state = ext_bt_force(i, off[rr], off_end[rr]);
            tmp = force_state < 0 ? p[(int64_t)rr * n_col + i - off[rr]] : 0;
        }
        state = ext_bt_next_state(state, tmp, force_state);
        if (state == 0) { MPN_PUSHOP(0, 1); --i; --j; }
        else if (state == 1 || state == 3) { MPN_PUSHOP(2, 1); --i; }
        else { MPN_PUSHOP(1, 1); --j; }
    }
    if (walk) {
        if (i >= 0) MPN_PUSHOP(2, (uint32_t)(i + 1));
        if (j >= 0) MPN_PUSHOP(1, (uint32_t)(j + 1));
        MPN_FLUSH();
    }
#undef MPN_PUSHOP
#undef MPN_FLUSH
    const int lane = threadIdx.x & 63;
    int incl = n;
#pragma unroll
    for (int d = 1; d < 64; d <<= 1) { const int o = __shfl_up(incl, d); if (lane >= d) incl += o; }
    const int total = __shfl(incl, 63);
    unsigned long long base = 0;
    if (lane == 0 && total) base = atomicAdd(compact_used, (unsigned long long)total);
    base = (unsigned long long)__shfl((long long)base, 0);
    if (walk) {
        const unsigned long long pos = base + (unsigned long long)(incl - n);
        const uint32_t *src = rev_cigar ? cbeg : cend - n;
        for (int q = 0; q < n; ++q) COMPACT[pos + q] = src[q];
        res[jid].n_cigar = n;
        res[jid].cig_pos = (int64_t)pos;
    }
}

__global__ __launch_bounds__(64) void ext_bt_wave_kernel(const ExtJob *__restrict__ jobs, const int32_t *__restrict__ order, int n_jobs,
                                                         const uint8_t *__restrict__ P, const int32_t *__restrict__ OFF,
                                                         uint32_t *__restrict__ CIG, uint32_t *__restrict__ COMPACT,
                                                         unsigned long long *__restrict__ compact_used, ExtRes *__restrict__ res,
                                                         unsigned long long *__restrict__ n_windows) {
    constexpr int PR = 64, PC = 64;
    __shared__ uint8_t patch[PR * PC];
    __shared__ int32_t s_lim[2][PR];
    const int lane = threadIdx.x;
    if ((int)blockIdx.x >= n_jobs) return;
    const int jid = order[blockIdx.x];
    if (jid < 0) return;
    if (lane == 0) atomicAdd(n_windows, 1ULL);
    const ExtJob jb = jobs[jid];
    const ExtRes r = res[jid];
    if (!r.do_bt) { if (lane == 0) res[jid].cig_pos = 0; return; }
    const int layout = jb.layout, S = jb.strip_s > 0 ? jb.strip_s : 1, R = 64 * S;
    const int n_col = jb.n_col, n_r = jb.qlen + jb.tlen - 1;
    const uint8_t *p = P + jb.p_off;
    const int32_t *off = OFF + 2 * jb.row_off, *off_end = off + n_r;
    const bool rank_is_op = (jb.flag & EZ_RIGHT) != 0 || layout == 0 || layout == 2;
    const int bw = jb.w < 0 ? (jb.tlen > jb.qlen ? jb.tlen : jb.qlen) : jb.w;
    const bool rev_cigar = (jb.flag & EZ_REV_CIGAR) != 0;
    uint32_t *cend = CIG + jb.cig_off;
    const int cap = jb.qlen + jb.tlen + 2;
    uint32_t *cbeg = cend - cap;
    int n = 0, i = r.bt_i, j = r.bt_j, state = 0;
    uint32_t cur_op = 0xf, cur_len = 0;
#define MPN_FLUSH() do { if (cur_len) { if (lane == 0) { if (rev_cigar) cbeg[n] = cur_len << 4 | cur_op; else cend[-1 - n] = cur_len << 4 | cur_op; } ++n; } } while (0)
#define MPN_PUSHOP(OP, LEN) do { if ((uint32_t)(OP) == cur_op) cur_len += (LEN); else { MPN_FLUSH(); cur_op = (OP); cur_len = (LEN); } } while (0)
    TileGeom tg{};
// ... 322 lines not shown
```

### megapath_nano_amd/csrc/mapper_internal.h

```cpp
#pragma once
#include "mpn_common.h"
#include "map_types.h"
#include "queue_lease.h"

#include <atomic>
#include <chrono>
#include <time.h>
#include <mutex>
#include <stdint.h>
#include <stdlib.h>
#include <string.h>
#include <string>
#include <vector>

struct mpn_map_opt_s;


struct mpn_index {
    int k = 15, w = 10;
    int32_t n_seq = 0;
    std::vector<std::string> names;
    std::vector<int32_t> lens;
    std::vector<int64_t> seq_off;
    std::vector<uint32_t> h_seq2;
    std::vector<int64_t> h_nrun_s, h_nrun_e;
    int64_t n_keys = 0, n_mz = 0;
    mpn::DevBuf<uint64_t> keys, pos;
    mpn::DevBuf<int64_t> key_off;
    mpn::DevBuf<int64_t> bucket_start;
    mpn::DevBuf<mpn::u128> kv;
    int bucket_shift = 0;
    mpn::DevBuf<uint32_t> d_seq2;
    mpn::DevBuf<int64_t> d_seq_off, d_nrun_s, d_nrun_e;
    mpn::DevBuf<int32_t> d_lens;
    int32_t n_nruns = 0;
    mutable std::mutex mu;
    mutable std::vector<std::pair<float, int32_t>> mid_occ_cache;
    mutable std::vector<uint64_t> occ_hist;
};

namespace mpn {

struct SeedChainOut {
    int64_t n_anchors = 0;
    DevBuf<unsigned char> tables;
    size_t tables_bytes = 0;
    DevBuf<int64_t> n_anchor;
    DevBuf<int64_t> anchor_off, c_off, n_chained, u_pos, b_pos;
    DevBuf<int32_t> rep_len, n_ends, n_chain;
    DevBuf<u128> anchors, chained;
    DevBuf<uint64_t> u, u_compact;
    DevBuf<ChainRec> recs;
    DevBuf<unsigned long long> used;
};

struct ReadSketch {
    DevBuf<int64_t> mz_off;
    DevBuf<u128> mz;
    int64_t n_mz = 0;
    int k = 0, w = 0;
    bool valid = false;
};

struct HostChains {
    std::vector<int64_t> n_anchor, chain_off, b_off;
    std::vector<int64_t> n_chained, u_pos, b_pos;
    std::vector<int32_t> n_chain, rep_len;
    const uint64_t *u_all = nullptr;
    const u128 *b_all = nullptr;
    const ChainRec *rec_all = nullptr;
    int64_t n_pool_chains = 0;
    void read_chains(int i, uint64_t *u_out, u128 *b_out) const;
    void chain_order(int i, int32_t *order, int64_t *src) const;
};

constexpr int MPN_NSTATS = 77;
constexpr int STAT_LEASE_WAIT = 65;
constexpr int STAT_SIDE_LEASED = 66, STAT_SIDE_OWN = 67;
constexpr int STAT_TILE_CLASS = 68, STAT_TILE_GIVEUPS = 72;
constexpr int STAT_WALK_WAVE = 73, STAT_EV_WALK_LONG = 74, STAT_WALK_WAVE_FAILED = 75;
constexpr int STAT_K_TAGS = 76;
extern thread_local int64_t g_stats[MPN_NSTATS];

void pack_2bit(const uint8_t *codes, int64_t n, std::vector<uint32_t> &words, std::vector<int64_t> &ns, std::vector<int64_t> &ne);

hipError_t stream_sync(hipStream_t st);

struct QueueStreams {
    LeasePool pool;
    std::vector<hipStream_t> st;
    explicit QueueStreams(int q) : pool(q), st((size_t)q, nullptr) {}
};
QueueStreams *queue_streams(int dev);

class StreamLease {
  public:
    explicit StreamLease(QueueStreams *qs) : qs_(qs) {}
    explicit StreamLease(hipStream_t fixed) : fixed_(fixed) {}
    StreamLease(const StreamLease &) = delete;
    StreamLease &operator=(const StreamLease &) = delete;
    ~StreamLease() { release(); }
    hipStream_t get() {
        if (!qs_) return fixed_;
        if (n_ == 0) n_ = qs_->pool.acquire(1, id_, &g_stats[STAT_LEASE_WAIT]);
        return qs_->st[(size_t)id_[0]];
    }
    operator hipStream_t() { return get(); }
    int try_extra(int k, hipStream_t *out) {
        if (!qs_ || n_ == 0) return 0;
        const int got = qs_->pool.try_acquire(std::min(k, 3 - n_), id_ + n_);
        for (int i = 0; i < got; ++i) out[i] = qs_->st[(size_t)id_[n_ + i]];
        n_ += got;
        return got;
    }
    hipError_t sync_release() {
        hipError_t rc = hipSuccess;
        if (!qs_) return stream_sync(fixed_);
        for (int i = 0; i < n_; ++i) { const hipError_t r = stream_sync(qs_->st[(size_t)id_[i]]); if (rc == hipSuccess) rc = r; }
        release();
        return rc;
    }

  private:
    void release() { if (qs_ && n_) { qs_->pool.release(id_, n_); n_ = 0; } }
    QueueStreams *qs_ = nullptr;
    hipStream_t fixed_ = nullptr;
    int id_[3] = {0, 0, 0};
    int n_ = 0;
};
static inline hipError_t stream_sync(StreamLease &st) { return st.sync_release(); }

struct EvTimer {
    hipStream_t st = nullptr;
    StreamLease *lease = nullptr;
    std::vector<hipEvent_t> ev;
    std::vector<int> slot, slot2;
    static bool enabled() { static const bool on = []() { const char *e = getenv("MPN_KERNEL_EVENTS"); return !e || atoi(e) != 0; }(); return on; }
    explicit EvTimer(hipStream_t s) : st(s) { push(); }
    explicit EvTimer(StreamLease &l) : lease(&l) { push(); }
    void push() {
        if (!enabled()) return;
        hipEvent_t e = nullptr;
        (void)hipEventCreate(&e);
        (void)hipEventRecord(e, lease ? lease->get() : st);
        ev.push_back(e);
        slot.push_back(-1); slot2.push_back(-1);
    }
    void mark(int stat_index, int single = -1) { if (!enabled()) return; slot.back() = stat_index; slot2.back() = single; push(); }
    void skip() { push(); }
    void resolve() {
        if (!enabled()) return;
        for (size_t i = 0; i + 1 < ev.size(); ++i) {
            if (slot[i] < 0 && slot2[i] < 0) continue;
            float ms = 0;
            if (hipEventElapsedTime(&ms, ev[i], ev[i + 1]) != hipSuccess) continue;
            if (slot[i] >= 0) g_stats[slot[i]] += (int64_t)(ms * 1e6);
            if (slot2[i] >= 0) g_stats[slot2[i]] += (int64_t)(ms * 1e6);
        }
        for (size_t i = 0; i + 1 < ev.size(); ++i) (void)hipEventDestroy(ev[i]);
        hipEvent_t last = ev.back();
        ev.assign(1, last); slot.assign(1, -1); slot2.assign(1, -1);
    }
    ~EvTimer() { for (hipEvent_t e : ev) (void)hipEventDestroy(e); }
};

struct PoolBuf {
    void *p = nullptr;
    size_t cap = 0;
    bool pinned_host = false;
    int ensure(size_t bytes) {
        if (bytes <= cap) return 0;
        if (p) { if (pinned_host) (void)hipHostFree(p); else (void)hipFree(p); p = nullptr; cap = 0; }
        size_t want = bytes + bytes / 8 + 4096;
        const hipError_t e_ = pinned_host ? hipHostMalloc(&p, want, hipHostMallocDefault) : guarded_malloc(&p, want);
        if (e_ != hipSuccess) {
            if (e_ == hipErrorOutOfMemory && !pinned_host) tl_oom = true;
            p = nullptr;
            set_error("%s of %zu bytes failed: %s", pinned_host ? "hipHostMalloc" : "hipMalloc", want, hipGetErrorString(e_));
            (void)hipGetLastError();
            return -1;
        }
        cap = want;
        return 0;
    }
    void release() { if (p) { if (pinned_host) (void)hipHostFree(p); else (void)hipFree(p); } p = nullptr; cap = 0; }
    template <typename T> T *as() const { return (T *)p; }
};

struct PhaseLog {
    struct Rec { int worker, slot; int64_t t0, t1; };
    std::mutex mu;
    std::vector<Rec> recs;
    bool on = false;
    std::chrono::steady_clock::time_point origin;
    void add(int worker, int slot, std::chrono::steady_clock::time_point a, std::chrono::steady_clock::time_point b) {
        std::lock_guard<std::mutex> g(mu);
        recs.push_back({worker, slot, std::chrono::duration_cast<std::chrono::nanoseconds>(a - origin).count(),
                        std::chrono::duration_cast<std::chrono::nanoseconds>(b - origin).count()});
    }
};
extern PhaseLog g_phase_log;
extern thread_local int tl_worker_id;

extern bool g_worker_cpu_on;
extern std::atomic<long long> g_worker_cpu_ns[64];
static inline long long thread_cpu_ns() {
    timespec t;
    clock_gettime(CLOCK_THREAD_CPUTIME_ID, &t);
    return t.tv_sec * 1000000000LL + t.tv_nsec;
}

struct WallTimer {
    std::chrono::steady_clock::time_point t0 = std::chrono::steady_clock::now();
    long long c0 = g_worker_cpu_on ? thread_cpu_ns() : 0;
    void stop_into(int64_t &acc) {
        auto t1 = std::chrono::steady_clock::now();
        acc += std::chrono::duration_cast<std::chrono::nanoseconds>(t1 - t0).count();
        if (g_phase_log.on) g_phase_log.add(tl_worker_id, (int)(&acc - g_stats), t0, t1);
        if (g_worker_cpu_on) { const long long c1 = thread_cpu_ns(); g_worker_cpu_ns[(&acc - g_stats) & 63] += c1 - c0; c0 = c1; }
        t0 = t1;
    }
};

}
```

### megapath_nano_amd/csrc/plan_kernels.h

```cpp
#pragma once
#include "stitch_kernels.h"

namespace mpn {

constexpr uint64_t PK_SEED_LONG_JOIN = 1ULL << 40, PK_SEED_IGNORE = 1ULL << 41, PK_SEED_TANDEM = 1ULL << 42;

struct PlanOpt {
    int32_t bw, bw15, min_chain_score, max_gap, min_cnt, a, q, e, zdrop, zdrop_inv, end_bonus, min_ksw_len, k, pad;
    int64_t max_sw_mat;
};

__device__ __forceinline__ int32_t pk_x(const u128 &v) { return (int32_t)v.x; }
__device__ __forceinline__ int32_t pk_y(const u128 &v) { return (int32_t)v.y; }
__device__ __forceinline__ int32_t pk_span(const u128 &v) { return (int32_t)(v.y >> 32 & 0xff); }

struct AnchorView {
    u128 *g;
    u128 *l;
    int lo, hi;
    const unsigned long long *kb;
    int kb_n;
    __device__ __forceinline__ u128 operator[](int i) const { return (i >= lo && i < hi) ? l[i - lo] : g[i]; }
    __device__ __forceinline__ void or_y(int i, uint64_t f) { g[i].y |= f; if (i >= lo && i < hi) l[i - lo].y |= f; }
};
// ... 143 lines not shown
        if (x > re0 && y > qe0) {
            if (++l > o.min_cnt) {
                l = x - re0 > y - qe0 ? x - re0 : y - qe0;
                re1 = re0 + l; qe1 = qe0 + l;
                break;
            }
        }
    }
    if (qe < qlen && re < tlen_all) {
        l = qlen - qe < o.max_gap ? qlen - qe : o.max_gap;
        qe1 = qe1 < qe + l ? qe1 : qe + l;
        qe0 = qe0 > qe1 ? qe0 : qe1;
        l += l * o.a > o.q ? (l * o.a - o.q) / o.e : 0;
        l = l < o.max_gap ? l : o.max_gap;
        l = l < tlen_all - re ? l : tlen_all - re;
        re1 = re1 < re + l ? re1 : re + l;
        re0 = re0 > re1 ? re0 : re1;
    } else { re0 = re; qe0 = qe; }
    const int32_t first_qs = qs, first_rs = rs;
    if (qs > 0 && rs > 0) {
        if (!too_big(qs - qs0, rs - rs0))
            emit(qs0, qs - qs0, rs0, rs - rs0, 1, bw, pr.split_inv ? o.zdrop_inv : o.zdrop, o.end_bonus, EZ_EXTZ_ONLY | EZ_RIGHT | EZ_REV_CIGAR, -1);
        else emit(qs0, 0, rs0, 0, 1, 0, 0, 0, EZ_EXTZ_ONLY | EZ_RIGHT | EZ_REV_CIGAR | EZ_REFUSED, -1);
    }
    for (i = 1; i < cnt1; ++i) {
        const uint64_t fl = a[as1 + i].y;
        if ((fl & (PK_SEED_IGNORE | PK_SEED_TANDEM)) && i != cnt1 - 1) continue;
        re = pk_x(a[as1 + i]) - kh; qe = pk_y(a[as1 + i]) - kh;
        if (i == cnt1 - 1 || (fl & PK_SEED_LONG_JOIN) || (qe - qs >= o.min_ksw_len && re - rs >= o.min_ksw_len)) {
            int bw1 = bw;
            if (fl & PK_SEED_LONG_JOIN) bw1 = qe - qs > re - rs ? qe - qs : re - rs;
            if (!too_big(qe - qs, re - rs) && qe - qs > 0 && re - rs > 0) emit(qs, qe - qs, rs, re - rs, 0, bw1, o.zdrop, -1, EZ_APPROX_MAX, i);
            else emit(qs, 0, rs, 0, 0, 0, 0, 0, EZ_APPROX_MAX | EZ_REFUSED, i);
            rs = re; qs = qe;
        }
    }
    if (qe < qe0 && re < re0) {
        if (!too_big(qe0 - qe, re0 - re)) emit(qe, qe0 - qe, re, re0 - re, 0, bw, o.zdrop, o.end_bonus, EZ_EXTZ_ONLY, -1);
        else emit(qe, 0, re, 0, 0, 0, 0, 0, EZ_EXTZ_ONLY | EZ_REFUSED, -1);
    }
    if constexpr (FILL) {
        sregs[ri] = StitchReg{first_job, nj, first_qs, first_rs, qe, re, qs0, qe0, pr.read, rid, rev, 0};
        psum[ri] = PlanSum{as1, cnt1};
    }
    return nj;
}

constexpr int PLAN_LDS_ANCHORS = 1024;
constexpr int PLAN_KBITS = 8192;
__global__ __launch_bounds__(64) void plan_kernel(PlanOpt o, const PlanReg *__restrict__ pregs, int n_regs, u128 *__restrict__ A,
                                                  const int32_t *__restrict__ tlens, unsigned long long *__restrict__ n_jobs_total,
                                                  ExtJob *__restrict__ jobs, int32_t *__restrict__ job_anchor, StitchReg *__restrict__ sregs,
                                                  PlanSum *__restrict__ psum) {
    __shared__ u128 lds_a[PLAN_LDS_ANCHORS];
    __shared__ unsigned long long lds_kb[PLAN_KBITS / 64];
    const int lane = threadIdx.x;
    for (int ri = blockIdx.x; ri < n_regs; ri += gridDim.x) {
        const PlanReg pr = pregs[ri];
        AnchorView av;
        av.g = A + pr.a_off; av.l = lds_a; av.lo = pr.as; av.hi = pr.as + (pr.cnt < PLAN_LDS_ANCHORS ? pr.cnt : PLAN_LDS_ANCHORS);
        av.kb = lds_kb; av.kb_n = pr.cnt < PLAN_KBITS ? pr.cnt : PLAN_KBITS;
        for (int i = lane; i < av.hi - av.lo; i += 64) lds_a[i] = av.g[av.lo + i];
        __syncthreads();
        for (int r0 = 0; r0 < av.kb_n; r0 += 64) {
            const int r = r0 + lane;
            bool big = false;
            if (r >= 1 && r < av.kb_n) {
                const u128 cur = av[av.lo + r], prev = av[av.lo + r - 1];
                const int gp = (pk_y(cur) - pk_y(prev)) - (pk_x(cur) - pk_x(prev));
                big = gp < -10 || gp > 10;
            }
            const unsigned long long m = __ballot(big);
            if (lane == 0) lds_kb[r0 >> 6] = m;
        }
        __syncthreads();
        if (lane == 0) {
            const int nj = plan_hit<false>(o, pr, av, tlens, ri, 0, jobs, job_anchor, sregs, psum);
            const int32_t first = (int32_t)atomicAdd(n_jobs_total, (unsigned long long)nj);
            plan_hit<true>(o, pr, av, tlens, ri, first, jobs, job_anchor, sregs, psum);
        }
        __syncthreads();
    }
}

constexpr int TILE_EXACT_MAX_NR = 4096;
constexpr int N_TILE_CLASS = 4;
__host__ __device__ inline int tile_class_s(int c) { return c == 0 ? 16 : c == 2 ? 8 : 4; }
__host__ __device__ inline int tile_class_nw(int c) { return c == 0 ? 1 : c == 1 ? 8 : c == 2 ? 4 : 16; }
constexpr int TILE_AUTO_CLASS = 1;
constexpr int TILE_LDS_CAP = 160 << 10;

constexpr int N_STRIP_CLASS = 9;
enum { L_LDS = 0, L_WG = 5, L_STRIP = 20, N_STRIP = 16 * N_STRIP_CLASS, L_BAND = L_STRIP + N_STRIP, L_TILE = L_BAND + 16, N_LISTS = L_TILE + N_TILE_CLASS };
constexpr int STRIP_QB = 64;
constexpr int N_BUCKETS = N_LISTS + N_STRIP * (STRIP_QB - 1);
__host__ __device__ inline int strip_glc_of_list(int l) { return ((l - L_STRIP) / 16) % 3; }
__host__ __device__ inline int strip_windows_per_wave(int l) { return (l < L_STRIP + 48 ? 8 : 4) >> strip_glc_of_list(l); }
__host__ __device__ inline int bucket_of_list(int l) {
    return l < L_STRIP ? l : l < L_BAND ? L_STRIP + (l - L_STRIP) * STRIP_QB : L_STRIP + N_STRIP * STRIP_QB + (l - L_BAND);
}

struct LayoutTotals {
    long long p_tot, row_tot, cig_tot, state_tot, cells, strip_cells[3], xstrip_cells;
    int lds_need[5], strip_lds[N_STRIP_CLASS], band_lds[4], strip_nr[N_STRIP_CLASS];
    int tile_lds[N_TILE_CLASS];
    int too_large, tl_q, tl_t, n_jobs;
    int cnt[N_LISTS], base[N_LISTS + 1];
};

struct JobSizes { long long p, row, cig, st; };

__global__ __launch_bounds__(256) void job_classify_kernel(ExtJob *__restrict__ jobs, const unsigned long long *__restrict__ nj_p, int strip_scores,
                                                           ExtParams prm, int force_kernel, int tile_pick, JobSizes *__restrict__ sizes,
                                                           int32_t *__restrict__ bucket_cnt, LayoutTotals *__restrict__ tot) {
    const int nj = (int)*nj_p;
    const bool no_tile = force_kernel == 7;
    if (no_tile) force_kernel = 0;
    const int lds_cap[4] = {8 << 10, 24 << 10, 64 << 10, 150 << 10};
    __shared__ int s_bucket[N_BUCKETS];
    constexpr int M_STRIP = 5, M_BAND = M_STRIP + N_STRIP_CLASS, M_NR = M_BAND + 4, M_TILE = M_NR + N_STRIP_CLASS, M_END = M_TILE + N_TILE_CLASS;
    __shared__ int s_max[M_END];
    for (int k = threadIdx.x; k < N_BUCKETS; k += blockDim.x) s_bucket[k] = 0;
    if (threadIdx.x < M_END) s_max[threadIdx.x] = 0;
    __syncthreads();
    long long cells = 0, scells[3] = {0, 0, 0}, xcells = 0;
    for (int j = blockIdx.x * blockDim.x + threadIdx.x; j < nj; j += gridDim.x * blockDim.x) {
        ExtJob jb = jobs[j];
        JobSizes sz{0, 0, 0, 0};
        if (jb.flag & EZ_REFUSED) { jb.cls = -1; jobs[j].cls = -1; sizes[j] = sz; continue; }
        const int w = jb.w < 0 ? max(jb.tlen, jb.qlen) : jb.w;
        int n_col = min(jb.qlen, jb.tlen);
        n_col = min(n_col, w + 1) + 1;
        jb.n_col = n_col;
        const long long n_r = (long long)jb.qlen + jb.tlen - 1;
        int glc = -1, variant = 0;
        if (w >= max(jb.qlen, jb.tlen) && strip_scores && (force_kernel == 0 || force_kernel == 4)) {
            bool fits = false;
            if (jb.flag & EZ_APPROX_MAX) fits = !(jb.flag & (EZ_EXTZ_ONLY | EZ_RIGHT)) && !jb.reversed;
            else {
                fits = ext_strip_exact_ok(prm.sc_mch, prm.q, prm.e, prm.q2, prm.e2, jb.qlen, jb.tlen);
                variant = (jb.flag & EZ_RIGHT) ? 2 : 1;
            }
            for (int c = 0; c < 3 && fits && glc < 0; ++c)
                if (jb.tlen <= (256 << c) && jb.qlen <= (1024 << c)) glc = c;
        }
        const bool strip = glc >= 0;
        const bool tile_exact = !(jb.flag & EZ_APPROX_MAX);
        int tcls = -1;
        if (!strip && strip_scores && !no_tile && (force_kernel == 0 || force_kernel == 6) &&
            (tile_exact ? ext_tile_exact_ok(prm.sc_mch, prm.sc_mis, prm.sc_n, prm.q, prm.e, prm.q2, prm.e2, jb.qlen, jb.tlen, w)
                        : (!(jb.flag & (EZ_EXTZ_ONLY | EZ_RIGHT)) && !jb.reversed && ext_tile_ok(jb.qlen, jb.tlen, w)))) {
            const int c = tile_pick < 0 ? TILE_AUTO_CLASS : tile_pick;
            if (c > 0 && ext_tile_pipe_ok(w, tile_class_s(c), tile_class_nw(c)) &&
                ext_tile_lds_bytes(jb.qlen, jb.tlen, tile_exact, tile_class_nw(c)) <= TILE_LDS_CAP) tcls = c;
            else if (!tile_exact || force_kernel == 6 || jb.qlen + jb.tlen <= TILE_EXACT_MAX_NR) tcls = 0;
        }
        const bool tiled = tcls >= 0;
        const int sclass = variant * 3 + max(glc, 0);
        const int seqb = ((jb.qlen + 3) & ~3) + ((jb.tlen + 3) & ~3);
        int bv = n_col <= 128 ? 0 : n_col <= 256 ? 1 : n_col <= 512 ? 2 : n_col <= 1024 ? 3 : -1;
        if (seqb > lds_cap[3] || !(force_kernel == 0 || force_kernel == 4 || force_kernel == 5)) bv = -1;
        int bc = 3;
        for (int c = 0; c < 4; ++c) if (seqb <= lds_cap[c]) { bc = c; break; }
        if (bv >= 0) atomicMax(&s_max[M_BAND + bc], seqb);
        jb.layout = strip ? 1 : tiled ? 3 : bv >= 0 ? 2 : 0;
        const int strip_gl = 16 << max(glc, 0);
        jb.strip_s = max(1, min(16, (jb.tlen + strip_gl - 1) / strip_gl));
        if (tiled) jb.strip_s = tile_class_s(tcls);
        const int strip_lanes = (jb.tlen + jb.strip_s - 1) / jb.strip_s;
        jb.qstride = strip ? strip_lanes * jb.strip_s : 128 << max(bv, 0);
        const long long strip_bytes = (long long)(jb.qlen + strip_lanes - 1) * (strip_lanes * jb.strip_s);
        sz.p = ((strip ? strip_bytes : tiled ? (long long)tile_matrix_bytes(jb.qlen, jb.tlen, w, jb.strip_s) : bv >= 0 ? n_r * (128 << bv) : n_r * n_col) + 15) & ~15LL;
        cells += n_r * n_col;
        if (strip) { if (variant == 0) scells[glc] += (long long)jb.qlen * jb.tlen; else xcells += (long long)jb.qlen * jb.tlen; }
        const int stateb = ((6 * jb.tlen + 3) & ~3) + 4 * jb.tlen;
        int cls = 4;
        for (int c = 0; c < 4; ++c) if (seqb + stateb <= lds_cap[c]) { cls = c; break; }
        jb.state_mode = 0;
        int wgc = n_col - 1 <= 128 ? 0 : n_col - 1 <= 256 ? 1 : n_col - 1 <= 512 ? 2 : 3;
        if (force_kernel == 1) wgc = 0;
        else if (force_kernel == 3) wgc = max(wgc, 1);
        const int redo_list = bv >= 0 ? L_BAND + bv * 4 + bc : L_LDS + wgc * 5 + cls;
        int lid;
        if (strip) {
            lid = L_STRIP + sclass * 16 + (16 - jb.strip_s);
            atomicMax(&s_max[M_STRIP + sclass], (jb.qlen + 15) & ~15);
            if (variant) atomicMax(&s_max[M_NR + sclass], (int)n_r);
        }
        else if (tiled) {
            lid = L_TILE + tcls;
            atomicMax(&s_max[M_TILE + tcls], ext_tile_lds_bytes(jb.qlen, jb.tlen, tile_exact, tile_class_nw(tcls)));
            sz.st = ((tcls == 0 ? (long long)24 * jb.qlen : 0) + (tile_exact ? (long long)4 * jb.tlen : 0) + 15) & ~15LL;
        }
        else if (bv >= 0) lid = L_BAND + bv * 4 + bc;
        else lid = redo_list;
        if (bv < 0) {
            if (cls == 4) {
                if (seqb > lds_cap[3]) { tot->too_large = 1; tot->tl_q = jb.qlen; tot->tl_t = jb.tlen; }
                jb.state_mode = 1; sz.st = max(sz.st, (long long)((stateb + 15) & ~15));
                atomicMax(&s_max[4], seqb);
            } else atomicMax(&s_max[cls], seqb + stateb);
            sz.row = n_r;
        }
        sz.cig = jb.qlen + jb.tlen + 2;
        jb.cls = lid | redo_list << 8 | (bv + 1) << 16;
        jobs[j] = jb;
        sizes[j] = sz;
        int b = bucket_of_list(lid);
        if (strip) b += STRIP_QB - 1 - min(STRIP_QB - 1, jb.qlen >> (4 + glc));
        atomicAdd(&s_bucket[b], 1);
    }
    __syncthreads();
    for (int k = threadIdx.x; k < N_BUCKETS; k += blockDim.x) if (s_bucket[k]) atomicAdd(&bucket_cnt[k], s_bucket[k]);
    if (threadIdx.x < M_END && s_max[threadIdx.x]) {
        const int k = threadIdx.x;
        atomicMax(k < M_STRIP ? &tot->lds_need[k] : k < M_BAND ? &tot->strip_lds[k - M_STRIP] : k < M_NR ? &tot->band_lds[k - M_BAND] :
                  k < M_TILE ? &tot->strip_nr[k - M_NR] : &tot->tile_lds[k - M_TILE], s_max[k]);
    }
    __shared__ long long red[5];
    if (threadIdx.x < 5) red[threadIdx.x] = 0;
    __syncthreads();
    long long v[5] = {cells, scells[0], scells[1], scells[2], xcells};
    for (int q = 0; q < 5; ++q) {
        for (int d = 32; d; d >>= 1) v[q] += __shfl_xor(v[q], d);
        if ((threadIdx.x & 63) == 0 && v[q]) atomicAdd((unsigned long long *)&red[q], (unsigned long long)v[q]);
    }
    __syncthreads();
    if (threadIdx.x == 0) {
        if (red[0]) atomicAdd((unsigned long long *)&tot->cells, (unsigned long long)red[0]);
        for (int c = 0; c < 3; ++c) if (red[1 + c]) atomicAdd((unsigned long long *)&tot->strip_cells[c], (unsigned long long)red[1 + c]);
        if (red[4]) atomicAdd((unsigned long long *)&tot->xstrip_cells, (unsigned long long)red[4]);
    }
}

__global__ __launch_bounds__(1024) void job_scan_kernel(JobSizes *__restrict__ sizes, const unsigned long long *__restrict__ nj_p,
                                                        const int32_t *__restrict__ bucket_cnt, int32_t *__restrict__ bucket_cur,
                                                        LayoutTotals *__restrict__ tot, int32_t *__restrict__ order) {
    __shared__ long long part[1024][4];
    __shared__ int list_cnt[N_LISTS], list_base[N_LISTS + 1];
    const int nj = (int)*nj_p;
    if (threadIdx.x == 0) tot->n_jobs = nj;
    const int t = threadIdx.x, per = (nj + 1023) / 1024, lo = min(nj, t * per), hi = min(nj, lo + per);
    long long s[4] = {0, 0, 0, 0};
    for (int j = lo; j < hi; ++j) { s[0] += sizes[j].p; s[1] += sizes[j].row; s[2] += sizes[j].cig; s[3] += sizes[j].st; }
    for (int q = 0; q < 4; ++q) part[t][q] = s[q];
    __syncthreads();
    if (t < 4) {
        long long acc = 0;
        for (int k = 0; k < 1024; ++k) { const long long v = part[k][t]; part[k][t] = acc; acc += v; }
        if (t == 0) tot->p_tot = acc; else if (t == 1) tot->row_tot = acc; else if (t == 2) tot->cig_tot = acc; else tot->state_tot = acc;
    }
    __syncthreads();
    long long o[4] = {part[t][0], part[t][1], part[t][2], part[t][3]};
    for (int j = lo; j < hi; ++j) {
        const JobSizes z = sizes[j];
        sizes[j] = JobSizes{o[0], o[1], o[2] + z.cig, o[3]};
        o[0] += z.p; o[1] += z.row; o[2] += z.cig; o[3] += z.st;
    }
    if (t < N_LISTS) {
        const int b0 = bucket_of_list(t), nb = (t >= L_STRIP && t < L_BAND) ? STRIP_QB : 1;
        int c = 0;
        for (int b = 0; b < nb; ++b) c += bucket_cnt[b0 + b];
        list_cnt[t] = c;
    }
    __syncthreads();
    if (t == 0) {
        int pos = 0;
        for (int l = 0; l < N_LISTS; ++l) {
            int c = list_cnt[l];
            list_base[l] = pos;
            if (l >= L_STRIP && l < L_BAND) { const int pw = strip_windows_per_wave(l); c = (c + pw - 1) / pw * pw; }
            pos += c;
        }
        list_base[N_LISTS] = pos;
    }
    __syncthreads();
    if (t < N_LISTS) {
        const int b0 = bucket_of_list(t), nb = (t >= L_STRIP && t < L_BAND) ? STRIP_QB : 1;
        int pos = list_base[t];
        for (int b = 0; b < nb; ++b) { bucket_cur[b0 + b] = pos; pos += bucket_cnt[b0 + b]; }
        tot->cnt[t] = list_cnt[t]; tot->base[t] = list_base[t];
        for (int k = list_base[t] + list_cnt[t]; k < list_base[t + 1]; ++k) order[k] = -1;
    }
    if (t == 0) tot->base[N_LISTS] = list_base[N_LISTS];
}

__global__ __launch_bounds__(256) void job_layout_kernel(ExtJob *__restrict__ jobs, const unsigned long long *__restrict__ nj_p,
                                                         const JobSizes *__restrict__ offs, int32_t *__restrict__ bucket_cur, int32_t *__restrict__ order) {
    const int nj = (int)*nj_p;
    for (int j = blockIdx.x * blockDim.x + threadIdx.x; j < nj; j += gridDim.x * blockDim.x) {
        ExtJob &jb = jobs[j];
        if (jb.cls < 0) continue;
        const JobSizes z = offs[j];
        jb.p_off = z.p; jb.row_off = z.row; jb.cig_off = z.cig; jb.state_off = z.st;
        const int lid = jb.cls & 0xff;
        int b = bucket_of_list(lid);
        if (lid >= L_STRIP && lid < L_BAND) b += STRIP_QB - 1 - min(STRIP_QB - 1, jb.qlen >> (4 + strip_glc_of_list(lid)));
        order[atomicAdd(&bucket_cur[b], 1)] = j;
    }
}

}
```

### megapath_nano_amd/mapper.py

```python
import ctypes as ct
import os

import numpy as np

from . import _ffi


class MapOpt(ct.Structure):
    _fields_ = [('k', ct.c_int32), ('w', ct.c_int32), ('mid_occ_frac', ct.c_float), ('mid_occ', ct.c_int32),
                ('max_gap', ct.c_int32), ('bw', ct.c_int32), ('max_chain_skip', ct.c_int32), ('max_chain_iter', ct.c_int32),
                ('min_cnt', ct.c_int32), ('min_chain_score', ct.c_int32), ('mask_level', ct.c_float),
                ('pri_ratio', ct.c_float), ('best_n', ct.c_int32), ('max_join_long', ct.c_int32),
                ('max_join_short', ct.c_int32), ('min_join_flank_sc', ct.c_int32), ('min_join_flank_ratio', ct.c_float),
                ('a', ct.c_int32), ('b', ct.c_int32), ('q', ct.c_int32), ('e', ct.c_int32), ('q2', ct.c_int32),
                ('e2', ct.c_int32), ('sc_ambi', ct.c_int32), ('zdrop', ct.c_int32), ('zdrop_inv', ct.c_int32),
                ('end_bonus', ct.c_int32), ('min_dp_max', ct.c_int32), ('min_ksw_len', ct.c_int32),
                ('max_clip_ratio', ct.c_float), ('max_sw_mat', ct.c_int64), ('with_cigar', ct.c_int32),
                ('seed', ct.c_uint32), ('host_threads', ct.c_int32), ('out_sam', ct.c_int32), ('out_tags', ct.c_int32)]


TAG_CS, TAG_CS_LONG, TAG_MD, TAG_EQX = 1, 2, 4, 8


COL_NAMES = ('read_idx', 'qs', 'qe', 'rev', 'rid', 'rs', 're', 'mlen', 'blen', 'mapq', 'nm', 'as_', 'primary')
# ... 730 lines not shown
    for c, o in zip(cigars, coff):
        cig[o:o + len(c)] = np.asarray(c, dtype=np.uint32)
    cols = sum(int(x) >> 4 for c in cigars for x in c)
    ops = int(ncig.astype(np.int64).sum())
    want_cs, want_md, want_eqx = bool(out_tags & (TAG_CS | TAG_CS_LONG)), bool(out_tags & TAG_MD), bool(out_tags & TAG_EQX)
    cs_cap, md_cap, eqx_cap = caps if caps is not None else (3 * cols + 2 * ops + 16, 2 * cols + 2 * ops + 16 * n + 16, cols + ops + 16)
    cs = np.zeros(cs_cap if want_cs else 1, dtype=np.uint8)
    md = np.zeros(md_cap if want_md else 1, dtype=np.uint8)
    eqx = np.zeros(eqx_cap if want_eqx else 1, dtype=np.uint32)
    cs_off, md_off, eqx_off = (np.zeros(n + 1, dtype=np.int64) for _ in range(3))
    rc = lib.mpn_aln_tags_batch(n, qbuf.ctypes.data, qoff.ctypes.data, qlen.ctypes.data, qs.ctypes.data, qe.ctypes.data, rev.ctypes.data,
                                tbuf.ctypes.data, toff.ctypes.data, tlen.ctypes.data, ts.ctypes.data, cig.ctypes.data, coff.ctypes.data,
                                ncig.ctypes.data, int(out_tags), cs.ctypes.data, cs_cap if want_cs else 0, cs_off.ctypes.data,
                                md.ctypes.data, md_cap if want_md else 0, md_off.ctypes.data, eqx.ctypes.data, eqx_cap if want_eqx else 0,
                                eqx_off.ctypes.data)
    _ffi.check(rc, 'mpn_aln_tags_batch')
    res = []
    for i in range(n):
        res.append(dict(cs=cs[cs_off[i]:cs_off[i + 1]].tobytes().decode() if want_cs else None,
                        md=md[md_off[i]:md_off[i + 1]].tobytes().decode() if want_md else None,
                        eqx=[int(x) for x in eqx[eqx_off[i]:eqx_off[i + 1]]] if want_eqx else None))
    return res



def aln_finish_batch(opt, queries, q_ivals, revs, targets, t_starts, cigars, force_class=0):
    lib = _bind()
    n = len(queries)
    qbuf, qoff, qlen = pack_seqs([np.asarray(q, dtype=np.uint8) for q in queries])
    tbuf, toff, tlen = pack_seqs([np.asarray(t, dtype=np.uint8) for t in targets])
    qs = np.ascontiguousarray([iv[0] for iv in q_ivals], dtype=np.int32)
    qe = np.ascontiguousarray([iv[1] for iv in q_ivals], dtype=np.int32)
    rev = np.ascontiguousarray(np.broadcast_to(np.asarray(revs, dtype=np.int32), (n,)))
    ts = np.ascontiguousarray(np.broadcast_to(np.asarray(t_starts, dtype=np.int32), (n,)))
    ncig = np.array([len(c) for c in cigars], dtype=np.int32)
    coff = np.zeros(n, dtype=np.int64)
    if n > 1:
        coff[1:] = np.cumsum(ncig[:-1].astype(np.int64))
    cig = np.zeros(int(ncig.astype(np.int64).sum()) + 1, dtype=np.uint32)
    for c, o in zip(cigars, coff):
        cig[o:o + len(c)] = np.asarray(c, dtype=np.uint32)
    out = np.zeros((n, 8), dtype=np.int32)
    fixed = np.zeros_like(cig)
    rc = lib.mpn_aln_finish_batch(ct.byref(opt), n, qbuf.ctypes.data, qoff.ctypes.data, qlen.ctypes.data, qs.ctypes.data, qe.ctypes.data,
                                  rev.ctypes.data, tbuf.ctypes.data, toff.ctypes.data, tlen.ctypes.data, ts.ctypes.data, cig.ctypes.data,
                                  coff.ctypes.data, ncig.ctypes.data, int(force_class), out.ctypes.data, fixed.ctypes.data)
    _ffi.check(rc, 'mpn_aln_finish_batch')
    keys = ('n_cigar', 'qshift', 'tshift', 'blen', 'mlen', 'n_ambi', 'dp_max')
    res = []
    for i in range(n):
        d = {k: int(out[i, j]) for j, k in enumerate(keys)}
        d['cigar'] = fixed[coff[i]:coff[i] + d['n_cigar']].tolist()
        res.append(d)
    return res


HIT_KEYS = ('fx', 'fy', 'lx', 'ly', 'score', 'score0', 'cnt', 'as', 'parent', 'subsc', 'n_sub', 'mlen', 'blen', 'hash', 'sam_pri')


def hit_select_batch(opt, k, q_len, names, chain_off, u, recs, anchor_off, anchors, path=0, max_chains=0, grid_cap=0):
    lib = _bind()
    n = len(q_len)
    c = lambda v, t: np.ascontiguousarray(v, dtype=t)
    q_len, chain_off, anchor_off, u = c(q_len, np.int32), c(chain_off, np.int64), c(anchor_off, np.int64), c(u, np.uint64)
    fx, fy, lx, ly = (c(r, np.uint64) for r in recs[:4])
    mlen, blen = c(recs[4], np.int32), c(recs[5], np.int32)
    anchors = c(anchors, np.uint64).reshape(-1, 2)
    assert len(chain_off) == n + 1 and len(anchor_off) == n + 1 and len(names) == n
    n_chains, n_anch = int(chain_off[-1]) if n else 0, int(anchor_off[-1]) if n else 0
    assert all(len(x) == n_chains for x in (u, fx, fy, lx, ly, mlen, blen)) and len(anchors) == n_anch
    cnames = (ct.c_char_p * max(1, n))(*[(nm.encode() if isinstance(nm, str) else nm) for nm in names])
    n_regs, n_a = np.zeros(n, dtype=np.int32), np.zeros(n, dtype=np.int32)
    hits = np.zeros((n_chains + 1, 15), dtype=np.int64)
    sq = np.zeros((n_anch + 1, 2), dtype=np.uint64)
    rc = lib.mpn_hit_select_batch(ct.byref(opt), int(k), n, q_len.ctypes.data, cnames, chain_off.ctypes.data, u.ctypes.data, fx.ctypes.data,
                                  fy.ctypes.data, lx.ctypes.data, ly.ctypes.data, mlen.ctypes.data, blen.ctypes.data, anchor_off.ctypes.data,
                                  anchors.ctypes.data, int(path), int(max_chains), int(grid_cap), n_regs.ctypes.data, n_a.ctypes.data,
                                  hits.ctypes.data, sq.ctypes.data)
    _ffi.check(rc, 'mpn_hit_select_batch')
    return n_regs, n_a, hits[:int(n_regs.sum())], (sq[:int(n_a.sum())] if opt.with_cigar else None)


PLAN_HIT_KEYS = ('n_jobs', 'as1', 'cnt1', 'qs', 'rs', 'qe', 're', 'qs0', 'qe0', 'rid', 'rev')
PLAN_WIN_KEYS = ('read', 'rid', 'rev', 'qs', 'qlen', 'ts', 'tlen', 'reversed', 'w', 'zdrop', 'end_bonus', 'flag', 'anchor')


def ext_plan_batch(opt, k, t_len, q_len, anchor_off, anchors, hit_off, h_as, h_cnt, h_mlen, h_split_inv, grid_cap=0):
    lib = _bind()
    n = len(q_len)
    c = lambda v, t: np.ascontiguousarray(v, dtype=t)
    t_len, q_len, anchor_off, hit_off = c(t_len, np.int32), c(q_len, np.int32), c(anchor_off, np.int64), c(hit_off, np.int64)
    h_as, h_cnt, h_mlen, h_split_inv = (c(v, np.int32) for v in (h_as, h_cnt, h_mlen, h_split_inv))
    anchors = c(anchors, np.uint64).reshape(-1, 2)
    assert len(anchor_off) == n + 1 and len(hit_off) == n + 1
    n_anch, n_hits = (int(anchor_off[-1]), int(hit_off[-1])) if n else (0, 0)
    assert len(anchors) == n_anch and all(len(v) == n_hits for v in (h_as, h_cnt, h_mlen, h_split_inv))
    win_cap = int(np.maximum(h_cnt.astype(np.int64), 0).sum()) + n_hits
    hits = np.zeros((n_hits + 1, 11), dtype=np.int32)
    wins = np.zeros((win_cap + 1, 13), dtype=np.int32)
    left = np.zeros((n_anch + 1, 2), dtype=np.uint64)
    n_win = ct.c_int64(0)
    rc = lib.mpn_ext_plan_batch(ct.byref(opt), int(k), len(t_len), t_len.ctypes.data, n, q_len.ctypes.data, anchor_off.ctypes.data,
                                anchors.ctypes.data, hit_off.ctypes.data, h_as.ctypes.data, h_cnt.ctypes.data, h_mlen.ctypes.data,
                                h_split_inv.ctypes.data, int(grid_cap), hits.ctypes.data, win_cap, ct.addressof(n_win), wins.ctypes.data,
                                left.ctypes.data)
    _ffi.check(rc, 'mpn_ext_plan_batch')
    return hits[:n_hits], wins[:n_win.value], left[:n_anch]


STITCH_HIT_KEYS = ('read', 'rid', 'rev', 'as', 'cnt', 'as1', 'cnt1', 'qs', 'rs', 'qe', 're', 'qs0', 'qe0', 'first_win', 'n_win')
STITCH_WIN_KEYS = ('flag', 'reversed', 'qs', 'ts', 'anchor', 'max', 'zdropped', 'max_q', 'max_t', 'mqe_t', 'score', 'reach_end', 'n_cigar')
STITCH_OUT_KEYS = ('cig_off', 'n_ops', 'dp_score', 'rs1', 're1', 'qs1', 'qe1', 'has_p', 'dropped', 'drop_fill', 'drop_max_t', 'drop_max_q',
                   'split_n', 'split_inv', 'split_rec')
STITCH_FIN_KEYS = ('cig_off', 'code_off', 'n_cigar', 'read', 'rid', 'rev', 'qs1', 'rs1', 'qspan', 'tspan')
STITCH_SPLIT_KEYS = ('fx', 'fy', 'lx_left', 'ly_left', 'mlen_l', 'blen_l', 'mlen_r', 'blen_r')


def stitch_batch(anchor_off, anchors, hits, wins, cig_pos, compact, min_cnt, grid_cap=0):
    lib = _bind()
    c = lambda v, t: np.ascontiguousarray(v, dtype=t)
    anchor_off, cig_pos, compact = c(anchor_off, np.int64), c(cig_pos, np.int64), c(compact, np.uint32)
    anchors, hits, wins = c(anchors, np.uint64).reshape(-1, 2), c(hits, np.int32).reshape(-1, 15), c(wins, np.int32).reshape(-1, 13)
    n = len(anchor_off) - 1
    assert n >= 0 and len(anchors) == (int(anchor_off[-1]) if n else 0) and len(cig_pos) == len(wins)
    n_hits = len(hits)
    pool_cap = int(np.maximum(wins[:, 12].astype(np.int64), 0).sum())
    out = np.zeros((n_hits + 1, 25), dtype=np.int64)
    pool = np.zeros(pool_cap + 1, dtype=np.uint32)
    splits = np.zeros((n_hits + 1, 8), dtype=np.int64)
    used, n_splits = ct.c_int64(0), ct.c_int64(0)
    rc = lib.mpn_stitch_batch(n, anchor_off.ctypes.data, anchors.ctypes.data, n_hits, hits.ctypes.data, len(wins), wins.ctypes.data,
                              cig_pos.ctypes.data, len(compact), compact.ctypes.data, int(min_cnt), int(grid_cap), out.ctypes.data, pool_cap,
                              pool.ctypes.data, ct.addressof(used), splits.ctypes.data, ct.addressof(n_splits))
    _ffi.check(rc, 'mpn_stitch_batch')
    return out[:n_hits], pool[:used.value], splits[:n_splits.value]


STAT_NAMES = {0: 'bases', 1: 'minimizers', 2: 'anchors', 3: 'chains', 4: 'dp_jobs', 5: 'dp_cells', 6: 'alignments',
              7: 'dp_rounds', 8: 'second_pass_jobs', 10: 'ev_sketch_ns', 11: 'ev_seed_ns', 12: 'ev_sort_ns',
              13: 'ev_chain_dp_ns', 14: 'ev_chain_bt_ns', 15: 'ev_ext_dp_ns', 25: 'ev_ext_bt_ns', 26: 'ev_ext_ztest_ns',
              16: 'wall_h2d_ns', 17: 'wall_seed_chain_ns', 18: 'wall_d2h_chains_ns', 19: 'wall_host_hits_ns',
              20: 'wall_host_plan_ns', 21: 'wall_ext_stage_ns', 22: 'wall_host_stitch_ns', 23: 'wall_host_final_ns',
              24: 'wall_total_ns', 27: 'wall_ext_host_prep_ns', 28: 'wall_ext_enqueue_ns', 29: 'wall_ext_gpu_wait_ns',
              30: 'wall_ext_finish_ns', 9: 'ev_ext_strip_ns', 31: 'strip_cells', 32: 'sub_batches',
              33: 'k_sketch_count_ns', 34: 'k_sketch_fill_ns', 35: 'k_seed_lookup_ns', 36: 'k_seed_fill_ns',
              37: 'k_chain_dp_ns', 38: 'k_strip16_ns', 39: 'k_strip32_ns', 40: 'k_strip64_ns', 41: 'strip16_cells',
              42: 'strip32_cells', 43: 'strip64_cells', 44: 'sort_records_moved', 45: 'anchors_kept', 46: 'k_compact_ns', 47: 'k_sort_msd_ns', 48: 'k_sort_chunk_ns', 49: 'k_sort_radix_ns',
              50: 'k_seed_filter_ns', 51: 'anchors_emitted', 52: 'k_finish_ns', 53: 'cigar_ops', 54: 'k_stitch_ns', 55: 'k_plan_ns', 56: 'k_layout_ns', 57: 'k_xstrip_ns', 58: 'xstrip_cells', 59: 'anchors_squeezed', 60: 'workers_shed', 61: 'workers', 62: 'k_hit_select_ns', 63: 'reads_hits_on_host',
              64: 'tile_windows', 65: 'wall_lease_wait_ns', 66: 'ext_groups_side_leased', 67: 'ext_groups_side_own',
              68: 'tile_windows_1w_s16', 69: 'tile_windows_s4_nw8', 70: 'tile_windows_s8_nw4', 71: 'tile_windows_s4_nw16',
              72: 'tile_wait_giveups',
              73: 'walk_wave_windows', 74: 'ev_ext_walk_long_ns',
              75: 'walk_wave_failed',
              76: 'k_tags_ns'}


def last_stats():
    n = max(STAT_NAMES) + 1
    s = np.zeros(n, dtype=np.int64)
    _bind().mpn_map_last_stats_ex(s.ctypes.data, n)
    return {name: int(s[i]) for i, name in STAT_NAMES.items()}
```

Baseline: 14.89.

## Defer exact tiled DP diagonal-max and z-drop to separate kernels via 16-bit H spill

```diff
diff --git a/megapath_nano_amd/csrc/align.hip b/megapath_nano_amd/csrc/align.hip
--- a/megapath_nano_amd/csrc/align.hip
+++ b/megapath_nano_amd/csrc/align.hip
@@ -805,7 +805,7 @@
     prm.zdrop_inv = opt->zdrop_inv; prm.max_gap = opt->max_gap;
     const size_t order_cap = (size_t)nj + (size_t)N_STRIP * 8 + 16;
     if (SL.pool_sizes.ensure((size_t)nj * sizeof(JobSizes) + 16) || SL.pool_buckets.ensure((size_t)2 * N_BUCKETS * 4 + sizeof(LayoutTotals) + 16) ||
-        SL.pool_order.ensure(order_cap * 4) || SL.pin_res.ensure(sizeof(LayoutTotals) + 96) ||
+        SL.pool_order.ensure(order_cap * 4) || SL.pin_res.ensure(sizeof(LayoutTotals) + 128) ||
         SL.pool_redo_ids.ensure((size_t)nj * 4 + 16) || SL.pool_probes.ensure((size_t)nj * sizeof(InvProbe) + 16))
         return -1;
     struct { ExtJob *p; } d_jobs{dv.jobs};
@@ -818,7 +818,7 @@
         zero_list_push(z, d_bcnt, (size_t)2 * N_BUCKETS * 4 + sizeof(LayoutTotals));
         zero_list_push(z, dv.used + 1, 8);
         zero_list_push(z, dv.used + 5, 8);
-        zero_list_push(z, dv.used + 8, 16);
+        zero_list_push(z, dv.used + 8, 24);
         zero_list_push(z, dv.used + 7, 8);
         MPN_HIP_CHECK(zero_regions(z, st));
     }
@@ -950,6 +950,9 @@
             static_assert(N_TILE_CLASS == 4, "tile classes");
             if (c == 0) MPN_TILE_LAUNCH(16, 1); else if (c == 1) MPN_TILE_LAUNCH(4, 8); else if (c == 2) MPN_TILE_LAUNCH(8, 4); else MPN_TILE_LAUNCH(4, 16);
 #undef MPN_TILE_LAUNCH
+            hipLaunchKernelGGL(ext_tile_diag_kernel, dim3(n, TILE_DIAG_BLOCKS), dim3(TILE_DIAG_THREADS), 0, s, d_jobs.p, ord, n, (int)(c == 0),
+                               std::min(prm.q + prm.e, prm.q2 + prm.e2), gstate.p);
+            hipLaunchKernelGGL(ext_tile_zdrop_kernel, dim3(n), dim3(64), 0, s, d_jobs.p, ord, n, prm, (int)(c == 0), (const int8_t *)gstate.p, d_res.p, d_used + 10);
         } else {
             const int bvar = (l - L_BAND) / 4;
             const size_t lds = std::max<size_t>((size_t)T.band_lds[(l - L_BAND) % 4], 64);
@@ -1034,12 +1037,13 @@
     if (side_st != main_st) MPN_HIP_CHECK(hipStreamWaitEvent(main_st, SL.ev_b, 0));
     if (tile_st != main_st) MPN_HIP_CHECK(hipStreamWaitEvent(main_st, SL.ev_c, 0));
     unsigned long long *h_used = reinterpret_cast<unsigned long long *>(reinterpret_cast<char *>(SL.pin_res.p) + ((sizeof(LayoutTotals) + 15) & ~(size_t)15));
-    MPN_HIP_CHECK(hipMemcpyAsync(h_used, d_used, 80, hipMemcpyDeviceToHost, st));
+    MPN_HIP_CHECK(hipMemcpyAsync(h_used, d_used, 88, hipMemcpyDeviceToHost, st));
     wt.stop_into(g_stats[28]);
     MPN_HIP_CHECK(stream_sync(st));
     wt.stop_into(g_stats[29]);
     g_stats[STAT_WALK_WAVE] += (int64_t)h_used[8];
     g_stats[STAT_WALK_WAVE_FAILED] += (int64_t)h_used[9];
+    g_stats[STAT_TILE_DEFERRED] += (int64_t)h_used[10];
     if (h_used[7]) {
         g_stats[STAT_TILE_GIVEUPS] += (int64_t)h_used[7];
         set_error("%llu tiled DP windows gave up waiting for their hand-off", (unsigned long long)h_used[7]);
diff --git a/megapath_nano_amd/csrc/ext_kernels.h b/megapath_nano_amd/csrc/ext_kernels.h
--- a/megapath_nano_amd/csrc/ext_kernels.h
+++ b/megapath_nano_amd/csrc/ext_kernels.h
@@ -928,6 +928,13 @@
 }
 
 struct TileGeom { int T0, rows, n_lanes, W, jlo, jhi; int64_t base; };
+__device__ __forceinline__ void ext_bt_band(int rr, int qlen, int tlen, int bw, int &st, int &en) {
+    st = 0; en = tlen - 1;
+    if (st < rr - qlen + 1) st = rr - qlen + 1;
+    if (en > rr) en = rr;
+    if (st < (rr - bw + 1) >> 1) st = (rr - bw + 1) >> 1;
+    if (en > (rr + bw) >> 1) en = (rr + bw) >> 1;
+}
 __host__ __device__ inline TileGeom tile_geom(int tile, int qlen, int tlen, int w, int S) {
     const int R = 64 * S;
     TileGeom g{};
@@ -969,8 +976,18 @@
 }
 constexpr int TILE_RING_COLS = 2048, TILE_CTRL_BYTES = 4 * (2 * 16 + 4);
 __host__ __device__ inline int ext_tile_ring_off(int qlen) { return ((qlen + 3) & ~3) + 64 + TILE_CTRL_BYTES; }
-__host__ __device__ inline int ext_tile_lds_bytes(int qlen, int tlen, bool exact, int NW) {
-    return ext_tile_ring_off(qlen) + (NW > 1 ? 12 * TILE_RING_COLS : 0) + (exact ? 8 * ((qlen + tlen + 2) & ~3) : 0);
+__host__ __device__ inline int ext_tile_lds_bytes(int qlen, int NW) {
+    return ext_tile_ring_off(qlen) + (NW > 1 ? 12 * TILE_RING_COLS : 0);
+}
+struct TileExactScratch { int64_t hl, status, best, h, end; };
+__host__ __device__ inline TileExactScratch ext_tile_exact_scratch(int qlen, int tlen, int w, int S, bool one_wave) {
+    TileExactScratch x;
+    x.hl = one_wave ? (int64_t)24 * qlen : 0;
+    x.status = (x.hl + 4 * (int64_t)tlen + 15) & ~(int64_t)15;
+    x.best = x.status + 16;
+    x.h = (x.best + 4 * ((int64_t)qlen + tlen - 1) + 15) & ~(int64_t)15;
+    x.end = (x.h + 2 * tile_matrix_bytes(qlen, tlen, w, S) + 15) & ~(int64_t)15;
+    return x;
 }
 __host__ __device__ inline bool ext_tile_pipe_ok(int w, int S, int NW) {
     return 2 * w + 128 < NW * (TILE_RING_COLS / NW + 64 * S);
@@ -995,7 +1012,13 @@
     out.max = 0; out.zdropped = 0; out.max_q = out.max_t = out.mqe_t = -1; out.mqe = NEG_INF; out.score = NEG_INF;
     out.reach_end = 0; out.n_cigar = 0; out.r_done = -1; out.bt_i = out.bt_j = -1; out.do_bt = 0; out.zcode = 0; out.cig_pos = 0;
     if (!(EXACT ? ext_tile_exact_ok(prm.sc_mch, prm.sc_mis, prm.sc_n, prm.q, prm.e, prm.q2, prm.e2, qlen, tlen, w) : ext_tile_ok(qlen, tlen, w)) || -prm.sc_mis > 2 * (q + e) ||
-        (NW > 1 && !ext_tile_pipe_ok(w, S, NW))) { if (tid == 0) res[jid] = out; return; }
+        (NW > 1 && !ext_tile_pipe_ok(w, S, NW))) {
+        if (tid == 0) {
+            res[jid] = out;
+            if constexpr (EXACT) *reinterpret_cast<uint32_t *>(gstate + jb.state_off + ext_tile_exact_scratch(qlen, tlen, w, S, NW == 1).status) = 1u;
+        }
+        return;
+    }
     constexpr int RS = RIGHT ? 0 : 4, RA = RIGHT ? 1 : 3, RB = 2, RA2 = RIGHT ? 3 : 1, RB2 = RIGHT ? 4 : 0;
     const uint32_t sb_mch = (uint32_t)(8 * prm.sc_mch + RS + 128) & 0xff, sb_mis = (uint32_t)(8 * prm.sc_mis + RS + 128) & 0xff,
                    sb_n = (uint32_t)(8 * prm.sc_n + RS + 128) & 0xff;
@@ -1030,23 +1053,16 @@
     uint32_t *ctrl = reinterpret_cast<uint32_t *>(smem + ext_tile_ring_off(qlen) - TILE_CTRL_BYTES);
     uint32_t *ring = ctrl + TILE_CTRL_BYTES / 4;
     constexpr int C = TILE_RING_COLS / NW;
-    const int n_r = qlen + tlen - 1;
-    uint32_t *BEST = reinterpret_cast<uint32_t *>(smem + ext_tile_ring_off(qlen) + (NW > 1 ? 12 * TILE_RING_COLS : 0)), *SE = BEST + ((n_r + 3) & ~3);
-    int32_t *HL = reinterpret_cast<int32_t *>(NW > 1 ? bnd_base : bnd_base + 6 * (size_t)qlen);
+    const TileExactScratch X = EXACT ? ext_tile_exact_scratch(qlen, tlen, w, S, NW == 1) : TileExactScratch{};
+    uint16_t *const H16 = reinterpret_cast<uint16_t *>(gstate + jb.state_off + X.h);
     if (tid < 2 * NW + 1) ctrl[tid] = 0;
     if constexpr (EXACT) {
-        for (int r = tid; r < n_r; r += NT) {
-            int st = 0, en = tlen - 1;
-            if (st < r - qlen + 1) st = r - qlen + 1;
-            if (en > r) en = r;
-            if (st < (r - w + 1) >> 1) st = (r - w + 1) >> 1;
-            if (en > (r + w) >> 1) en = (r + w) >> 1;
-            if (st > en) { st = 1; en = 0; }
-            BEST[r] = 0;
-            SE[r] = (uint32_t)st | (uint32_t)en << 16;
-        }
+        const int n_r = qlen + tlen - 1;
+        uint32_t *BEST = reinterpret_cast<uint32_t *>(gstate + jb.state_off + X.best);
+        int32_t *HL = reinterpret_cast<int32_t *>(gstate + jb.state_off + X.hl);
+        for (int r = tid; r < n_r; r += NT) BEST[r] = 0;
         for (int t = tid; t < tlen; t += NT) HL[t] = NEG_INF;
-        __builtin_amdgcn_fence(__ATOMIC_RELEASE, "agent");
+        if (tid == 0) *reinterpret_cast<uint32_t *>(gstate + jb.state_off + X.status) = 0u;
     }
     __syncthreads();
     const bool head = lane == 0;
@@ -1088,6 +1104,7 @@
             H8[k] = 8 * (t < long_thres ? -(q + e * (t + 1)) : -(q2 + e2 * (t + 1)));
         }
         uint8_t *prow = P + jb.p_off + G.base + (int64_t)lane * S;
+        uint16_t *hrow = H16 + G.base + (int64_t)lane * S;
         const int n_steps = (jhi - jlo + 1) + n_lanes - 1;
         int out_v = 0, out_x = 0, out_h = 0;
         uint32_t qt = 0;
@@ -1128,7 +1145,7 @@
                 else { Vp = bv; Xp = bx; Hup = (int32_t)bh; }
             } else { Vp = (uint32_t)v_s; Xp = (uint32_t)x_s; Hup = h_s; }
             if (j >= jlo && j <= jhi && lane < n_lanes) {
-                uint32_t dw[S / 4], ecell[4] = {0, 0, 0, 0};
+                uint32_t dw[S / 4], ecell[4] = {0, 0, 0, 0}, hw[S / 2], h_even = 0;
                 const int d_in = j - t0 + w;
                 const int d_out = j - t0 - w;
 #pragma unroll
@@ -1166,15 +1183,8 @@
                     H8[k] = h;
                     Hup = h;
                     if constexpr (EXACT) {
-                        const int t = t0 + k, r = t + j;
-                        const uint32_t se = SE[r < n_r ? r : n_r - 1];
-                        const int st_ = (int)(se & 0xffffu), en_ = (int)(se >> 16);
-                        const bool inb = t >= st_ && t <= en_;
-                        const int en1 = st_ + ((en_ - st_) & ~3);
-                        const int cls = t == en_ ? 0 : t < en1 ? 1 + ((t - st_) & 3) : 5;
-                        const uint32_t word = (uint32_t)((h >> 3) + 32768) << 16 | (0xffffu - ((uint32_t)cls << 13 | (uint32_t)t));
-                        atomicMax(&BEST[r < n_r ? r : n_r - 1], inb ? word : 0u);
-                        if (inb && j == qlen - 1) HL[t] = h >> 3;
+                        if (k & 1) hw[k >> 1] = ((uint32_t)h << 13 & 0xffff0000u) | h_even;
+                        else h_even = (uint32_t)h >> 3 & 0xffffu;
                     }
                     UL[k] = nu; YL[k] = __builtin_bit_cast(uint32_t, Bn);
                     Vp = nv; Xp = __builtin_bit_cast(uint32_t, An);
@@ -1190,6 +1200,14 @@
                 if constexpr (S == 16) *reinterpret_cast<uint4 *>(prow + (int64_t)step * W) = make_uint4(dw[0], dw[1], dw[2], dw[3]);
                 else if constexpr (S == 8) *reinterpret_cast<uint2 *>(prow + (int64_t)step * W) = make_uint2(dw[0], dw[1]);
                 else if constexpr (S == 4) *reinterpret_cast<uint32_t *>(prow + (int64_t)step * W) = dw[0];
+                if constexpr (EXACT) {
+                    uint16_t *hp = hrow + (int64_t)step * W;
+                    if constexpr (S == 4) *reinterpret_cast<uint2 *>(hp) = make_uint2(hw[0], hw[1]);
+                    else {
+#pragma unroll
+                        for (int k = 0; k < S / 8; ++k) reinterpret_cast<uint4 *>(hp)[k] = make_uint4(hw[4 * k], hw[4 * k + 1], hw[4 * k + 2], hw[4 * k + 3]);
+                    }
+                }
                 if constexpr (NW == 1) {
                     if (write_bnd && lane == 63) { bnd_out[3 * (size_t)j] = (uint32_t)out_v; bnd_out[3 * (size_t)j + 1] = (uint32_t)out_x; bnd_out[3 * (size_t)j + 2] = (uint32_t)out_h; }
                 } else if (write_bnd && lane == 63 && j >= jlo_next) {
@@ -1220,12 +1238,14 @@
     }
 #undef MPN_BND
     if constexpr (NW > 1) {
-        __builtin_amdgcn_fence(__ATOMIC_RELEASE, "agent");
         __syncthreads();
-        __builtin_amdgcn_fence(__ATOMIC_ACQUIRE, "agent");
         if (wave != (EXACT ? 0 : (n_tiles - 1) % NW)) return;
         if (__hip_atomic_load(&ctrl[2 * NW], __ATOMIC_RELAXED, __HIP_MEMORY_SCOPE_WORKGROUP)) {
-            if (lane == 0) { res[jid] = out; atomicAdd(n_failed, 1ull); }
+            if (lane == 0) {
+                res[jid] = out;
+                atomicAdd(n_failed, 1ull);
+                if constexpr (EXACT) *reinterpret_cast<uint32_t *>(gstate + jb.state_off + X.status) = 1u;
+            }
             return;
         }
     }
@@ -1234,66 +1254,6 @@
             out.score = score8 >> 3;
             out.r_done = qlen + tlen - 2;
             out.do_bt = 1; out.bt_i = tlen - 1; out.bt_j = qlen - 1;
-            res[jid] = out;
-        }
-    } else {
-        if constexpr (NW == 1) __syncthreads();
-        const int tlm1 = tlen - 1;
-        struct Best { int m, t, r; };
-        auto scan_first_max = [&](Best x) {
-#pragma unroll
-            for (int d = 1; d < 64; d <<= 1) {
-                const Best o{__shfl_up(x.m, d), __shfl_up(x.t, d), __shfl_up(x.r, d)};
-                if (lane >= d && !(x.m > o.m)) x = o;
-            }
-            return x;
-        };
-        auto diag = [&](int r, int &H, int &mt) {
-            const uint32_t pv = BEST[r];
-            H = pv ? (int)(pv >> 16) - 32768 : NEG_INF;
-            mt = (int)((0xffffu - (pv & 0xffffu)) & 8191u);
-        };
-        int r_lim = n_r;
-        for (int r = lane; r < n_r; r += 64) { const uint32_t se = SE[r]; if ((int)(se & 0xffffu) > (int)(se >> 16)) { r_lim = r; break; } }
-        r_lim = wave_reduce_min(r_lim);
-        const int n_eff = r_lim < n_r ? r_lim : n_r;
-        const int C = (n_eff + 63) / 64, rlo = min(n_eff, lane * C), rhi = min(n_eff, rlo + C);
-        auto chunk_best = [&](int lim) {
-            Best b{NEG_INF, -1, -1};
-            for (int r = rlo; r < rhi && r <= lim; ++r) { int H, mt; diag(r, H, mt); if (H > b.m) b = Best{H, mt, r}; }
-            return b;
-        };
-        Best incl = scan_first_max(chunk_best(n_eff));
-        Best in{__shfl_up(incl.m, 1), __shfl_up(incl.t, 1), __shfl_up(incl.r, 1)};
-        ExtApply ez; ez.max = 0; ez.max_t = ez.max_q = -1; ez.zdropped = 0;
-        if (lane > 0 && in.m > 0) { ez.max = in.m; ez.max_t = in.t; ez.max_q = in.r - in.t; }
-        int r_break = n_eff;
-        for (int r = rlo; r < rhi; ++r) {
-            int H, mt; diag(r, H, mt);
-            if (ext_apply_zdrop(ez, H, r, mt, jb.zdrop, e2)) { r_break = r; break; }
-        }
-        r_break = wave_reduce_min(r_break);
-        const bool zd = r_break < n_eff;
-        const bool dropped = zd || n_eff < n_r;
-        const int r_last = zd ? r_break : n_eff - 1;
-        Best fin = scan_first_max(chunk_best(r_last));
-        fin = Best{__shfl(fin.m, 63), __shfl(fin.t, 63), __shfl(fin.r, 63)};
-        __builtin_amdgcn_fence(__ATOMIC_ACQUIRE, "agent");
-        const int t_lim = min(tlm1, r_last - (qlen - 1));
-        const int Ct = (tlen + 63) / 64, tlo = min(tlen, lane * Ct), thi = min(tlen, tlo + Ct);
-        Best me{NEG_INF, -1, -1};
-        for (int t = tlo; t < thi && t <= t_lim; ++t) { const int h = HL[t]; if (h > me.m) me = Best{h, t, t}; }
-        me = scan_first_max(me);
-        me = Best{__shfl(me.m, 63), __shfl(me.t, 63), 0};
-        if (lane == 0) {
-            if (fin.m > 0) { out.max = fin.m; out.max_t = fin.t; out.max_q = fin.r - fin.t; }
-            out.zdropped = dropped ? 1 : 0;
-            if (me.m > NEG_INF) { out.mqe = me.m; out.mqe_t = me.t; }
-            if (!dropped) out.score = HL[tlm1];
-            out.r_done = dropped ? (zd ? r_break : n_eff) : n_r - 1;
-            if (!dropped && !(jb.flag & EZ_EXTZ_ONLY)) { out.do_bt = 1; out.bt_i = tlen - 1; out.bt_j = qlen - 1; }
-            else if (!dropped && (jb.flag & EZ_EXTZ_ONLY) && out.mqe + jb.end_bonus > out.max) { out.reach_end = 1; out.do_bt = 1; out.bt_i = out.mqe_t; out.bt_j = qlen - 1; }
-            else if (out.max_t >= 0 && out.max_q >= 0) { out.do_bt = 1; out.bt_i = out.max_t; out.bt_j = out.max_q; }
             res[jid] = out;
         }
     }
@@ -1315,15 +1275,140 @@
 #undef MPN_TB
 }
 
-
-
-__device__ __forceinline__ void ext_bt_band(int rr, int qlen, int tlen, int bw, int &st, int &en) {
-    st = 0; en = tlen - 1;
-    if (st < rr - qlen + 1) st = rr - qlen + 1;
-    if (en > rr) en = rr;
-    if (st < (rr - bw + 1) >> 1) st = (rr - bw + 1) >> 1;
-    if (en > (rr + bw) >> 1) en = (rr + bw) >> 1;
-}
+constexpr int TILE_DIAG_BLOCKS = 64, TILE_DIAG_STEPS = 128, TILE_DIAG_THREADS = 256;
+__global__ __launch_bounds__(TILE_DIAG_THREADS) void ext_tile_diag_kernel(const ExtJob *__restrict__ jobs, const int32_t *__restrict__ order, int n_jobs,
+                                                                          int one_wave, int qe, int8_t *__restrict__ gstate) {
+    __shared__ uint32_t best[TILE_DIAG_STEPS + 64 * 16];
+    const int jid = order[blockIdx.x];
+    const ExtJob jb = jobs[jid];
+    if (jb.flag & EZ_APPROX_MAX) return;
+    const int qlen = jb.qlen, tlen = jb.tlen, S = jb.strip_s, R = 64 * S, tid = threadIdx.x;
+    const int w = jb.w < 0 ? (tlen > qlen ? tlen : qlen) : jb.w;
+    const TileExactScratch X = ext_tile_exact_scratch(qlen, tlen, w, S, one_wave != 0);
+    int8_t *const base = gstate + jb.state_off;
+    if (*reinterpret_cast<const uint32_t *>(base + X.status)) return;
+    const uint16_t *const H16 = reinterpret_cast<const uint16_t *>(base + X.h);
+    uint32_t *const BEST = reinterpret_cast<uint32_t *>(base + X.best);
+    int32_t *const HL = reinterpret_cast<int32_t *>(base + X.hl);
+    const int nt_all = (tlen + R - 1) / R, nt_band = (int)(((int64_t)qlen - 1 + w) / R) + 1, nt = nt_all < nt_band ? nt_all : nt_band;
+    int c_base = 0;
+    for (int tile = 0; tile < nt; ++tile) {
+        const TileGeom G = tile_geom(tile, qlen, tlen, w, S);
+        const int n_steps = (G.jhi - G.jlo + 1) + G.n_lanes - 1, n_chunks = (n_steps + TILE_DIAG_STEPS - 1) / TILE_DIAG_STEPS;
+        const int upr = G.W >> 2;
+        int c = ((int)blockIdx.y + TILE_DIAG_BLOCKS - c_base % TILE_DIAG_BLOCKS) % TILE_DIAG_BLOCKS;
+        c_base += n_chunks;
+        for (; c < n_chunks; c += TILE_DIAG_BLOCKS) {
+            const int s0 = c * TILE_DIAG_STEPS, s1 = s0 + TILE_DIAG_STEPS < n_steps ? s0 + TILE_DIAG_STEPS : n_steps;
+            const int r_base = G.T0 + G.jlo + s0;
+            const int span = (s1 - s0) + G.n_lanes * (S - 1);
+            for (int i = tid; i < span; i += TILE_DIAG_THREADS) best[i] = 0;
+            __syncthreads();
+            const int n_units = (s1 - s0) * upr;
+            for (int u = tid; u < n_units; u += TILE_DIAG_THREADS) {
+                const int ds = u / upr, cell0 = (u - ds * upr) << 2, step = s0 + ds;
+                const int j = G.jlo + step - cell0 / S;
+                if (j < G.jlo || j > G.jhi) continue;
+                const uint2 hv = *reinterpret_cast<const uint2 *>(H16 + G.base + (int64_t)step * G.W + cell0);
+#pragma unroll
+                for (int i = 0; i < 4; ++i) {
+                    const int t = G.T0 + cell0 + i, r = t + j;
+                    const uint32_t hword = i < 2 ? hv.x : hv.y;
+                    int H = (int)(int16_t)(i & 1 ? hword >> 16 : hword & 0xffffu);
+                    int st, en;
+                    ext_bt_band(r, qlen, tlen, w, st, en);
+                    if (t < st || t > en) continue;
+                    if (t == tlen - 1 && t > 0 && j == t + w) H += qe;
+                    const int en1 = st + ((en - st) & ~3);
+                    const int cls = t == en ? 0 : t < en1 ? 1 + ((t - st) & 3) : 5;
+                    atomicMax(&best[r - r_base], (uint32_t)(H + 32768) << 16 | (0xffffu - ((uint32_t)cls << 13 | (uint32_t)t)));
+                    if (j == qlen - 1) HL[t] = H;
+                }
+            }
+            __syncthreads();
+            for (int i = tid; i < span; i += TILE_DIAG_THREADS) { const uint32_t v = best[i]; if (v) atomicMax(&BEST[r_base + i], v); }
+            __syncthreads();
+        }
+    }
+}
+
+__global__ __launch_bounds__(64) void ext_tile_zdrop_kernel(const ExtJob *__restrict__ jobs, const int32_t *__restrict__ order, int n_jobs, ExtParams prm,
+                                                            int one_wave, const int8_t *__restrict__ gstate, ExtRes *__restrict__ res,
+                                                            unsigned long long *__restrict__ n_done) {
+    const int jid = order[blockIdx.x], lane = threadIdx.x;
+    const ExtJob jb = jobs[jid];
+    if (jb.flag & EZ_APPROX_MAX) return;
+    const int qlen = jb.qlen, tlen = jb.tlen;
+    const int w = jb.w < 0 ? (tlen > qlen ? tlen : qlen) : jb.w;
+    const TileExactScratch X = ext_tile_exact_scratch(qlen, tlen, w, jb.strip_s, one_wave != 0);
+    const int8_t *const base = gstate + jb.state_off;
+    if (*reinterpret_cast<const uint32_t *>(base + X.status)) return;
+    const uint32_t *const BEST = reinterpret_cast<const uint32_t *>(base + X.best);
+    const int32_t *const HL = reinterpret_cast<const int32_t *>(base + X.hl);
+    const int e2 = prm.q2 + prm.e2 < prm.q + prm.e ? prm.e : prm.e2;
+    ExtRes out;
+    out.max = 0; out.zdropped = 0; out.max_q = out.max_t = out.mqe_t = -1; out.mqe = NEG_INF; out.score = NEG_INF;
+    out.reach_end = 0; out.n_cigar = 0; out.r_done = -1; out.bt_i = out.bt_j = -1; out.do_bt = 0; out.zcode = 0; out.cig_pos = 0;
+    const int n_r = qlen + tlen - 1, tlm1 = tlen - 1;
+    struct Best { int m, t, r; };
+    auto scan_first_max = [&](Best x) {
+#pragma unroll
+        for (int d = 1; d < 64; d <<= 1) {
+            const Best o{__shfl_up(x.m, d), __shfl_up(x.t, d), __shfl_up(x.r, d)};
+            if (lane >= d && !(x.m > o.m)) x = o;
+        }
+        return x;
+    };
+    auto diag = [&](int r, int &H, int &mt) {
+        const uint32_t pv = BEST[r];
+        H = pv ? (int)(pv >> 16) - 32768 : NEG_INF;
+        mt = (int)((0xffffu - (pv & 0xffffu)) & 8191u);
+    };
+    int r_lim = n_r;
+    for (int r = lane; r < n_r; r += 64) { int st, en; ext_bt_band(r, qlen, tlen, w, st, en); if (st > en) { r_lim = r; break; } }
+    r_lim = wave_reduce_min(r_lim);
+    const int n_eff = r_lim < n_r ? r_lim : n_r;
+    const int C = (n_eff + 63) / 64, rlo = min(n_eff, lane * C), rhi = min(n_eff, rlo + C);
+    auto chunk_best = [&](int lim) {
+        Best b{NEG_INF, -1, -1};
+        for (int r = rlo; r < rhi && r <= lim; ++r) { int H, mt; diag(r, H, mt); if (H > b.m) b = Best{H, mt, r}; }
+        return b;
+    };
+    Best incl = scan_first_max(chunk_best(n_eff));
+    Best in{__shfl_up(incl.m, 1), __shfl_up(incl.t, 1), __shfl_up(incl.r, 1)};
+    ExtApply ez; ez.max = 0; ez.max_t = ez.max_q = -1; ez.zdropped = 0;
+    if (lane > 0 && in.m > 0) { ez.max = in.m; ez.max_t = in.t; ez.max_q = in.r - in.t; }
+    int r_break = n_eff;
+    for (int r = rlo; r < rhi; ++r) {
+        int H, mt; diag(r, H, mt);
+        if (ext_apply_zdrop(ez, H, r, mt, jb.zdrop, e2)) { r_break = r; break; }
+    }
+    r_break = wave_reduce_min(r_break);
+    const bool zd = r_break < n_eff;
+    const bool dropped = zd || n_eff < n_r;
+    const int r_last = zd ? r_break : n_eff - 1;
+    Best fin = scan_first_max(chunk_best(r_last));
+    fin = Best{__shfl(fin.m, 63), __shfl(fin.t, 63), __shfl(fin.r, 63)};
+    const int t_lim = min(tlm1, r_last - (qlen - 1));
+    const int Ct = (tlen + 63) / 64, tlo = min(tlen, lane * Ct), thi = min(tlen, tlo + Ct);
+    Best me{NEG_INF, -1, -1};
+    for (int t = tlo; t < thi && t <= t_lim; ++t) { const int h = HL[t]; if (h > me.m) me = Best{h, t, t}; }
+    me = scan_first_max(me);
+    me = Best{__shfl(me.m, 63), __shfl(me.t, 63), 0};
+    if (lane == 0) {
+        if (fin.m > 0) { out.max = fin.m; out.max_t = fin.t; out.max_q = fin.r - fin.t; }
+        out.zdropped = dropped ? 1 : 0;
+        if (me.m > NEG_INF) { out.mqe = me.m; out.mqe_t = me.t; }
+        if (!dropped) out.score = HL[tlm1];
+        out.r_done = dropped ? (zd ? r_break : n_eff) : n_r - 1;
+        if (!dropped && !(jb.flag & EZ_EXTZ_ONLY)) { out.do_bt = 1; out.bt_i = tlen - 1; out.bt_j = qlen - 1; }
+        else if (!dropped && (jb.flag & EZ_EXTZ_ONLY) && out.mqe + jb.end_bonus > out.max) { out.reach_end = 1; out.do_bt = 1; out.bt_i = out.mqe_t; out.bt_j = qlen - 1; }
+        else if (out.max_t >= 0 && out.max_q >= 0) { out.do_bt = 1; out.bt_i = out.max_t; out.bt_j = out.max_q; }
+        res[jid] = out;
+        atomicAdd(n_done, 1ULL);
+    }
+}
+
 __device__ __forceinline__ int ext_bt_force(int i, int st, int en) {
     int force_state = -1;
     if (i < st) force_state = 2;
diff --git a/megapath_nano_amd/csrc/mapper_internal.h b/megapath_nano_amd/csrc/mapper_internal.h
--- a/megapath_nano_amd/csrc/mapper_internal.h
+++ b/megapath_nano_amd/csrc/mapper_internal.h
@@ -74,12 +74,13 @@
     void chain_order(int i, int32_t *order, int64_t *src) const;
 };
 
-constexpr int MPN_NSTATS = 77;
+constexpr int MPN_NSTATS = 78;
 constexpr int STAT_LEASE_WAIT = 65;
 constexpr int STAT_SIDE_LEASED = 66, STAT_SIDE_OWN = 67;
 constexpr int STAT_TILE_CLASS = 68, STAT_TILE_GIVEUPS = 72;
 constexpr int STAT_WALK_WAVE = 73, STAT_EV_WALK_LONG = 74, STAT_WALK_WAVE_FAILED = 75;
 constexpr int STAT_K_TAGS = 76;
+constexpr int STAT_TILE_DEFERRED = 77;
 extern thread_local int64_t g_stats[MPN_NSTATS];
 
 void pack_2bit(const uint8_t *codes, int64_t n, std::vector<uint32_t> &words, std::vector<int64_t> &ns, std::vector<int64_t> &ne);
diff --git a/megapath_nano_amd/csrc/plan_kernels.h b/megapath_nano_amd/csrc/plan_kernels.h
--- a/megapath_nano_amd/csrc/plan_kernels.h
+++ b/megapath_nano_amd/csrc/plan_kernels.h
@@ -319,7 +319,7 @@
                         : (!(jb.flag & (EZ_EXTZ_ONLY | EZ_RIGHT)) && !jb.reversed && ext_tile_ok(jb.qlen, jb.tlen, w)))) {
             const int c = tile_pick < 0 ? TILE_AUTO_CLASS : tile_pick;
             if (c > 0 && ext_tile_pipe_ok(w, tile_class_s(c), tile_class_nw(c)) &&
-                ext_tile_lds_bytes(jb.qlen, jb.tlen, tile_exact, tile_class_nw(c)) <= TILE_LDS_CAP) tcls = c;
+                ext_tile_lds_bytes(jb.qlen, tile_class_nw(c)) <= TILE_LDS_CAP) tcls = c;
             else if (!tile_exact || force_kernel == 6 || jb.qlen + jb.tlen <= TILE_EXACT_MAX_NR) tcls = 0;
         }
         const bool tiled = tcls >= 0;
@@ -356,8 +356,9 @@
         }
         else if (tiled) {
             lid = L_TILE + tcls;
-            atomicMax(&s_max[M_TILE + tcls], ext_tile_lds_bytes(jb.qlen, jb.tlen, tile_exact, tile_class_nw(tcls)));
-            sz.st = ((tcls == 0 ? (long long)24 * jb.qlen : 0) + (tile_exact ? (long long)4 * jb.tlen : 0) + 15) & ~15LL;
+            atomicMax(&s_max[M_TILE + tcls], ext_tile_lds_bytes(jb.qlen, tile_class_nw(tcls)));
+            sz.st = tile_exact ? (long long)ext_tile_exact_scratch(jb.qlen, jb.tlen, w, jb.strip_s, tcls == 0).end
+                               : ((tcls == 0 ? (long long)24 * jb.qlen : 0) + 15) & ~15LL;
         }
         else if (bv >= 0) lid = L_BAND + bv * 4 + bc;
         else lid = redo_list;
diff --git a/megapath_nano_amd/mapper.py b/megapath_nano_amd/mapper.py
--- a/megapath_nano_amd/mapper.py
+++ b/megapath_nano_amd/mapper.py
@@ -906,7 +906,8 @@
               72: 'tile_wait_giveups',
               73: 'walk_wave_windows', 74: 'ev_ext_walk_long_ns',
               75: 'walk_wave_failed',
-              76: 'k_tags_ns'}
+              76: 'k_tags_ns',
+              77: 'tile_windows_deferred'}
 
 
 def last_stats():
```

After: 15.12, median of 6. 1.02x the previous value.
